# mcosovic/JuliaGrid.jl

Measured on AMD Instinct MI355X. Metric: NR iterations/sec (batched N-1 AC power flow, 10k-bus grid), higher is better.
Workload: dtype f64

## Files before the change

### include/jgrid.h

```cpp
#ifndef JGRID_H
#define JGRID_H

#include <stdint.h>

#ifdef __cplusplus
extern "C" {
#endif

typedef struct jg_nr jg_nr;
typedef struct jg_nr_base jg_nr_base;
typedef struct jg_gn jg_gn;

const char* jg_last_error(void);
int jg_device_count(void);
void jg_plan_cache_clear(void);


int jg_nr_create(jg_nr** h, int64_t n, const int64_t* colptr, const int64_t* rowval,
                 const double* y_reim, const double* yt_reim, const int8_t* type, int64_t slack,
                 int64_t batch, int64_t max_patch, int device);
void jg_nr_destroy(jg_nr* h);

int jg_nr_dims(jg_nr* h, int64_t* dims);

int jg_nr_set_injection(jg_nr* h, const double* p_inj, const double* q_inj, int64_t batch_stride);
int jg_nr_set_voltage(jg_nr* h, const double* vm, const double* va, int64_t batch_stride);
int jg_nr_get_voltage(jg_nr* h, double* vm, double* va);
int jg_nr_snapshot_voltage(jg_nr* h);
int jg_nr_restore_voltage(jg_nr* h);
int jg_nr_get_voltage_device(jg_nr* h, double* vm_dev, double* va_dev);
int jg_nr_pack_results_device(jg_nr* h, double* dst_dev);

int jg_nr_patch_ybus(jg_nr* h, int64_t scenario, int64_t k, const int64_t* ptr, const double* dy_reim);

int jg_nr_patch_ybus_batch(jg_nr* h, int64_t scenario0, int64_t count, int64_t k, const int64_t* ptr, const double* dy_reim);

int jg_nr_set_ybus(jg_nr* h, const double* y_reim, const double* yt_reim);

int jg_nr_mismatch(jg_nr* h, double* max_p, double* max_q);
int jg_nr_solve(jg_nr* h);
int jg_nr_set_refine(jg_nr* h, int mode);
int jg_nr_set_shared(jg_nr* h, int mode);
int jg_nr_run(jg_nr* h, int64_t max_iter, double tol, int32_t* iters, int32_t* status);
int jg_nr_run_defer(jg_nr* h, int64_t max_iter, double tol, int64_t defer_at, int32_t* n_left);
int jg_nr_move_lanes(jg_nr* dst, int64_t dst_lane0, jg_nr* src, int32_t* home, int32_t* count);
int jg_nr_finish(jg_nr* h, int32_t* iters, int32_t* status);
int jg_nr_resume(jg_nr* h, int64_t lanes, int64_t max_iter, double tol, int32_t* iters, int32_t* status);
int jg_nr_pack_rows_device(jg_nr* h, double* dst_dev, int64_t lane0, int64_t count, const int32_t* rows);

int jg_nr_base_create(jg_nr_base** out, jg_nr* single, int64_t top_cap);
void jg_nr_base_destroy(jg_nr_base* b);
int jg_nr_base_info(jg_nr_base* b, int64_t* info);
int jg_nr_base_get(jg_nr_base* b, int which, double* out, int64_t cap);
int jg_nr_attach_base(jg_nr* h, jg_nr_base* b);
int jg_nr_start_from_base(jg_nr* h);
int jg_nr_set_first_iteration(jg_nr* h, int mode);
int jg_nr_first_iteration_counts(jg_nr* h, int64_t* compensated, int64_t* refactorised);

int jg_nr_get_mismatch(jg_nr* h, double* mism);
int jg_nr_get_increment(jg_nr* h, double* incr);
int jg_nr_get_jacobian(jg_nr* h, double* nzval);
int jg_nr_get_maps(jg_nr* h, int64_t* pq, int64_t* pvpq, int64_t* pcount, int64_t* jcolptr, int64_t* jrowval);
int jg_nr_get_iteration(jg_nr* h, int32_t* iters);

int jg_nr_set_bus_type(jg_nr* h, int64_t scenario0, int64_t count, const int8_t* type);
int jg_nr_get_bus_type(jg_nr* h, int8_t* type, int64_t* slack);

int jg_nr_set_generators(jg_nr* h, int64_t ng, const int64_t* bus, const int8_t* status, const double* pg, const double* qmin, const double* qmax,
                         const double* vg, const double* bus_vm, const double* bus_va, const double* pd, const double* qd, double base_mva);
int jg_nr_reactive_limit(jg_nr* h, int flags, int8_t* violate, int32_t* count);
int jg_nr_adjust_angle(jg_nr* h, int64_t bus, double angle);

int jg_nr_fast_setup(jg_nr* h, const double* bp, const double* bq);
int jg_nr_fast_patch_batch(jg_nr* h, int64_t scenario0, int64_t count, int64_t k, const int64_t* ptr, const double* dbp, const double* dbq);
int jg_nr_fast_mismatch(jg_nr* h, double* max_p, double* max_q);
int jg_nr_fast_solve(jg_nr* h);
int jg_nr_fast_run(jg_nr* h, int64_t max_iter, double tol, int32_t* iters, int32_t* status);
int jg_nr_fast_get_increment(jg_nr* h, double* incr);

int jg_nr_set_branches(jg_nr* h, int64_t nb, const int64_t* from, const int64_t* to, const int8_t* status, const double* param);
int jg_nr_set_outage_labels(jg_nr* h, const int64_t* label);
int jg_nr_branch_quantities(jg_nr* h, double* from_pq, double* to_pq, double* series_pq, double* charging_pq,
                            double* from_i, double* to_i, double* series_i);
int jg_nr_bus_injection(jg_nr* h, double* inj_pq);

int jg_nr_set_screen(jg_nr* h, const double* rating);
int jg_nr_screen(jg_nr* h, double* rec);
int jg_nr_screen_device(jg_nr* h, double* rec_dev);
int jg_nr_screen_rows_device(jg_nr* h, double* rec_dev, int64_t lane0, int64_t count, const int32_t* rows);

int jg_nr_time_kernel(jg_nr* h, int kernel, int reps, double* mean_ms);


int jg_gn_create(jg_gn** h, int64_t n, const int64_t* colptr, const int64_t* rowval, const double* y_reim,
                 const double* yt_reim, int64_t nb, const int64_t* from, const int64_t* to, const double* branch_param,
// ... 180 lines not shown
```

### juliagrid.jl_amd/_lib.py

```python
import ctypes as C
import os

import numpy as np

HERE = os.path.dirname(os.path.abspath(__file__))
LIB_PATH = os.environ.get("JG_LIB") or os.path.join(HERE, "libjgrid_hip.so")

I64P = np.ctypeslib.ndpointer(dtype=np.int64, flags="C_CONTIGUOUS")
I32P = np.ctypeslib.ndpointer(dtype=np.int32, flags="C_CONTIGUOUS")
I8P = np.ctypeslib.ndpointer(dtype=np.int8, flags="C_CONTIGUOUS")
F64P = np.ctypeslib.ndpointer(dtype=np.float64, flags="C_CONTIGUOUS")
U8P = np.ctypeslib.ndpointer(dtype=np.uint8, flags="C_CONTIGUOUS")
VP = C.c_void_p

_lib = None


class JGridError(RuntimeError):

    def __init__(self, code, msg):
        super().__init__(f"libjgrid_hip error {code}: {msg}")
        self.code = code


def lib():
    global _lib
    if _lib is not None:
        return _lib
    if not os.path.exists(LIB_PATH):
        raise ImportError(
            f"{LIB_PATH} is missing: build it with `python -c 'import __graft_entry__ as g; g.build()'` "
            "(hipcc --offload-arch=gfx950). There is no CPU fallback.")
    if not os.environ.get("JG_LIB") and not os.environ.get("JG_ALLOW_STALE"):
        from . import build as _build
        if _build.needs_build():
            raise ImportError(f"{LIB_PATH} was not built from the current csrc/ + include/jgrid.h (content hash differs or is missing): rebuild with "
                              "`python -c 'import __graft_entry__ as g; g.build()'`, or set JG_ALLOW_STALE=1 to load it anyway")
    L = C.CDLL(LIB_PATH)
    L.jg_last_error.restype = C.c_char_p
    L.jg_device_count.restype = C.c_int
    sig = {
        "jg_nr_create": [C.POINTER(VP), C.c_int64, I64P, I64P, F64P, F64P, I8P, C.c_int64, C.c_int64, C.c_int64, C.c_int],
        "jg_nr_dims": [VP, I64P],
        "jg_nr_set_injection": [VP, F64P, F64P, C.c_int64],
        "jg_nr_set_voltage": [VP, F64P, F64P, C.c_int64],
        "jg_nr_get_voltage": [VP, F64P, F64P],
        "jg_nr_snapshot_voltage": [VP],
        "jg_nr_restore_voltage": [VP],
        "jg_nr_get_voltage_device": [VP, VP, VP],
        "jg_nr_pack_results_device": [VP, VP],
        "jg_nr_patch_ybus": [VP, C.c_int64, C.c_int64, I64P, F64P],
        "jg_nr_patch_ybus_batch": [VP, C.c_int64, C.c_int64, C.c_int64, I64P, F64P],
        "jg_nr_set_ybus": [VP, F64P, F64P],
        "jg_nr_mismatch": [VP, F64P, F64P],
        "jg_nr_solve": [VP],
        "jg_nr_set_refine": [VP, C.c_int],
        "jg_nr_set_shared": [VP, C.c_int],
        "jg_nr_run": [VP, C.c_int64, C.c_double, I32P, I32P],
        "jg_nr_run_defer": [VP, C.c_int64, C.c_double, C.c_int64, C.POINTER(C.c_int32)],
        "jg_nr_move_lanes": [VP, C.c_int64, VP, I32P, C.POINTER(C.c_int32)],
        "jg_nr_finish": [VP, I32P, I32P],
        "jg_nr_resume": [VP, C.c_int64, C.c_int64, C.c_double, I32P, I32P],
        "jg_nr_pack_rows_device": [VP, VP, C.c_int64, C.c_int64, I32P],
        "jg_nr_get_mismatch": [VP, F64P],
        "jg_nr_get_increment": [VP, F64P],
        "jg_nr_get_jacobian": [VP, F64P],
        "jg_nr_get_maps": [VP, I64P, I64P, I64P, I64P, I64P],
        "jg_nr_get_iteration": [VP, I32P],
        "jg_nr_set_bus_type": [VP, C.c_int64, C.c_int64, VP],
        "jg_nr_get_bus_type": [VP, I8P, I64P],
        "jg_nr_set_generators": [VP, C.c_int64, I64P, I8P, F64P, F64P, F64P, F64P, F64P, F64P, F64P, F64P, C.c_double],
        "jg_nr_reactive_limit": [VP, C.c_int, VP, VP],
        "jg_nr_adjust_angle": [VP, C.c_int64, C.c_double],
        "jg_nr_time_kernel": [VP, C.c_int, C.c_int, C.POINTER(C.c_double)],
        "jg_nr_fast_setup": [VP, F64P, F64P],
        "jg_nr_fast_mismatch": [VP, F64P, F64P],
        "jg_nr_fast_solve": [VP],
        "jg_nr_fast_run": [VP, C.c_int64, C.c_double, I32P, I32P],
        "jg_nr_fast_get_increment": [VP, F64P],
        "jg_nr_set_branches": [VP, C.c_int64, I64P, I64P, I8P, F64P],
        "jg_nr_set_outage_labels": [VP, I64P],
        "jg_nr_branch_quantities": [VP, VP, VP, VP, VP, VP, VP, VP],
        "jg_nr_bus_injection": [VP, F64P],
        "jg_nr_set_screen": [VP, VP],
        "jg_nr_screen": [VP, F64P],
        "jg_nr_screen_device": [VP, VP],
        "jg_nr_screen_rows_device": [VP, VP, C.c_int64, C.c_int64, I32P],
        "jg_gn_create": [C.POINTER(VP), C.c_int64, I64P, I64P, F64P, F64P, C.c_int64, I64P, I64P, F64P, C.c_int64, C.c_int64,
                         I8P, I8P, I64P, C.c_int64, I64P, C.c_int64, C.c_int],
        "jg_gn_dims": [VP, I64P],
        "jg_gn_set_method": [VP, C.c_int],
        "jg_gn_set_measurement": [VP, F64P, F64P, F64P, C.c_int64, C.c_int64],
        "jg_gn_set_voltage": [VP, F64P, F64P, C.c_int64],
        "jg_gn_get_voltage": [VP, F64P, F64P],
        "jg_gn_snapshot_voltage": [VP],
        "jg_gn_restore_voltage": [VP],
        "jg_gn_increment": [VP, F64P],
        "jg_gn_solve": [VP],
        "jg_gn_residual_test": [VP, F64P, I32P],
        "jg_gn_get_normalized_residual": [VP, F64P],
        "jg_gn_evaluate": [VP],
        "jg_gn_set_status": [VP, I8P, I8P],
        "jg_gn_run": [VP, C.c_int64, C.c_double, I32P, I32P],
        "jg_gn_get_maps": [VP, I8P, I64P, I64P],
        "jg_gn_get_jacobian": [VP, F64P],
        "jg_gn_get_residual": [VP, F64P],
        "jg_gn_get_increment": [VP, F64P],
        "jg_gn_get_iteration": [VP, I32P],
        "jg_nr_fast_patch_batch": [VP, C.c_int64, C.c_int64, C.c_int64, I64P, F64P, F64P],
        "jg_gn_set_readings": [VP, C.c_int64, I64P, I8P, F64P, F64P, I8P, F64P, F64P, I8P],
# ... 250 lines not shown
```

### juliagrid.jl_amd/contingency.py

```python
from __future__ import annotations

import queue
import threading
from types import SimpleNamespace as NS

import numpy as np

from . import _lib
from .dcpowerflow import dcContingencyAnalysis
from .pipeline import OrderedRun, gatherBlocks
from .powerflow import (AcPowerFlow, BaseCase, fastNewtonRaphsonBX, fastNewtonRaphsonXB, newtonRaphson, powerFlow_, powerFlowLimits_, setBusType_, setInjection_,
                        setOutages_, startFromBase_, setFirstIteration_, _push_voltage, _upload_branches)
from .system import PowerSystem


def bridges(system: PowerSystem) -> np.ndarray:
    n, nb = system.bus.number, system.branch.number
    f = system.branch.layout.from_ - 1
    t = system.branch.layout.to - 1
    on = np.flatnonzero(system.branch.layout.status == 1)
    adj = [[] for _ in range(n)]
    for k in on:
        adj[f[k]].append((int(t[k]), int(k)))
        adj[t[k]].append((int(f[k]), int(k)))
# ... 187 lines not shown
        while not ev.wait(0.05):
            if run.failed:
                break
            if all(run.solved(i) for i in range(run.nj)):
                self.flush_filling()

    def _serve(self):
        try:
            while True:
                p = self.flush_q.get()
                if p is None:
                    return
                it, st = p.handle.resume(p.fill, self.iteration, self.tolerance)
                for j, home, off in p.routes:
                    result = self.run.wait_solved(j)
                    if result is None:
                        break
                    result[0][home] = it[off:off + home.size]
                    result[1][home] = st[off:off + home.size]
                    if self.record is not None:
                        if self.summary:
                            p.handle.screen_rows_device(self.record(j), off, home)
                        else:
                            p.handle.pack_rows_device(self.record(j), off, home)
                    self.pending[j].set()
                p.clear()
        except BaseException as e:
            self.run.fail(e)


class ContingencyPipeline:

    def __init__(self, system: PowerSystem, batch: int, inflight: int = 3, device: int = 0, start=None, pool: int = 0, defer_at: int = 64,
                 shared_first: bool = True, top_cap: int = 0, reactive_limit: int = 0):
        if reactive_limit and pool:
            raise ValueError("ContingencyPipeline: reactive_limit > 0 with a straggler pool (pool > 0) is not supported")
        if reactive_limit and int(batch) < 2:
            raise ValueError("ContingencyPipeline: reactive_limit needs batches of two or more scenarios")
        self.reactive_limit = max(0, int(reactive_limit))
        self.system, self.batch = system, int(batch)
        self.base = None
        self._shared_first, self._top_cap, self._device = bool(shared_first), int(top_cap), int(device)
        self.handles = [newtonRaphson(system, batch=self.batch, device=device, max_patch=4) for _ in range(max(1, int(inflight)))]
        self.defer_at = max(0, min(64, int(defer_at)))
        self.pools = []
        if pool and self.batch > 64 and self.defer_at > 0:
            lanes = max(2 * self.defer_at, -(-int(pool) // 64) * 64)
            lanes = max(lanes, 256) if -(-self.batch // 64) * 64 >= 256 else min(max(lanes, 128), 192)
            self.pools = [_Pool(newtonRaphson(system, batch=lanes, device=device, max_patch=4)) for _ in range(2)]
        self._stragglers = _StragglerPools(self.pools, self.defer_at) if self.pools else None
        if len(self.handles) + len(self.pools) > 1:
            for an in self.handles + [p.handle for p in self.pools]:
                _lib.check(_lib.lib().jg_nr_set_shared(an._h, 1))
        if start is not None:
            self.setStart(*start)
        else:
            for an in self.handles:
                an.snapshot_voltage()

    def setStart(self, magnitude, angle):
        for an in self.handles:
            _push_voltage(an, magnitude, angle)
            an.snapshot_voltage()
        for p in self.pools:
            _push_voltage(p.handle, magnitude, angle)
        if self.base is not None:
            self.base.close()
            self.base = None
        if self._shared_first and np.ndim(magnitude) == 1:
            single = newtonRaphson(self.system, batch=1, device=self._device)
            _push_voltage(single, magnitude, angle)
            self.base = BaseCase(single, top_cap=self._top_cap)
            single.close()
            for an in self.handles:
                self.base.attach(an)

    def setFirstIteration(self, shared: bool = True):
        for an in self.handles:
            setFirstIteration_(an, shared)

    def close(self):
        for an in self.handles:
            an.close()
        for p in self.pools:
            p.handle.close()
        if self.base is not None:
            self.base.close()
            self.base = None
        self.handles, self.pools, self._stragglers = [], [], None

    def setRating(self, rating):
        r = None if rating is None else np.ascontiguousarray(np.asarray(rating, dtype=np.float64))
        if r is not None and r.shape != (self.system.branch.number,):
            raise ValueError("rating: one value per branch")
        for an in self.handles + [p.handle for p in self.pools]:
            if not an._branches_on_device:
                _upload_branches(an)
            _lib.check(_lib.lib().jg_nr_set_screen(an._h, None if r is None else r.ctypes.data))
            an._screen_rating = r

    def run(self, jobs, iteration: int = 20, tolerance: float = 1e-8, on_done=None, fetch: bool = False, record=None, records: int = 0,
            summary: bool = False):
        jobs = list(jobs)
        pools = self._stragglers
        if pools is not None and on_done is not None and record is None:
            raise ValueError("a pipeline with a straggler pool delivers results through `record`")
# ... 85 lines not shown
```

### juliagrid.jl_amd/csrc/jg_comp.hip

```cpp
#include "jg_comp.hpp"
#include "jg_pf.hpp"

#include <algorithm>
#include <cstdio>
#include <cstdlib>

namespace jg {

namespace {

typedef int RecS __attribute__((ext_vector_type(16)));
typedef const RecS __attribute__((address_space(4)))* RecPtr;
typedef int SegS __attribute__((ext_vector_type(8)));
typedef const SegS __attribute__((address_space(4)))* SegPtr;
typedef const double __attribute__((address_space(4)))* CDbl;
typedef const int __attribute__((address_space(4)))* CInt;
__device__ __forceinline__ RecS load_rec(const Rec* base, size_t index) { return ((RecPtr)base)[index]; }

__device__ __forceinline__ void dsolve(double d00, double d01, double d10, double d11, double r1, double r2, double& y1, double& y2) {
    const bool sw = d10 > 2.0;
    const double l = sw ? d10 - 4.0 : d10;
    const double a = sw ? r2 : r1, b = sw ? r1 : r2;
    y2 = (b - l * a) * d11;
    y1 = (a - d01 * y2) * d00;
}

struct CSweepArgs {
    const Rec* rec; const Segment* seg;
    const double* Mc;
    const double* rhs;
    double* W;
    double* out;
    GroupSel sel; StateUpdate upd;
    int ld, seg_begin, lanes;
    int s0_base, s0_nchunks, s0_wpi, s0_rpw;
};

__device__ __forceinline__ void csweep_record(const CSweepArgs& a, const RecS& r, size_t ld, unsigned off, double& a0, double& a1) {
    static_assert(COMP_T == 6, "operand list of the wait");
    const int nt = r[3];
    d2v w[COMP_T];
#pragma unroll
    for (int t = 0; t < COMP_T; ++t) asm volatile("" : "=v"(w[t]));
#pragma unroll
    for (int t = 0; t < COMP_T; ++t)
        if (t < nt) gload16(w[t], (const char*)a.W + (size_t)r[5 + 2 * t] * ld * 16, off);
    asm volatile("s_waitcnt vmcnt(0)" ::: "memory");
    asm volatile("" : "+v"(w[0]), "+v"(w[1]), "+v"(w[2]), "+v"(w[3]), "+v"(w[4]), "+v"(w[5]));
#pragma unroll
    for (int t = 0; t < COMP_T; ++t)
        if (t < nt) {
            CDbl m = (CDbl)a.Mc + (size_t)r[4 + 2 * t] * 4;
            a0 = fma(-m[1], w[t].y, fma(-m[0], w[t].x, a0));
            a1 = fma(-m[3], w[t].y, fma(-m[2], w[t].x, a1));
        }
}

template <bool BWD>
__global__ __launch_bounds__(512, 4) void k_csweep(CSweepArgs a) {
    extern __shared__ __attribute__((aligned(16))) double red[];
    int base = a.s0_base, nchunks = a.s0_nchunks, wpi = a.s0_wpi, rpw = a.s0_rpw;
    if (blockIdx.y != 0) {
        const SegS sg = ((SegPtr)a.seg)[a.seg_begin + blockIdx.y];
        base = sg[0]; nchunks = sg[1]; wpi = sg[2]; rpw = sg[3];
    }
    int grp, bx;
    if (!map_block(a.sel, a.ld, nchunks * 2, grp, bx)) return;
    const int lane = threadIdx.x;
    const int wave = uniform(threadIdx.y);
    const size_t ld = (size_t)a.ld;
    const size_t b = (size_t)min(grp * 64 + lane, a.lanes - 1);
    const unsigned off = (unsigned)b * 16u;
    const size_t ri = (size_t)base + ((size_t)bx * 8 + wave) * rpw;
    const RecS first = load_rec(a.rec, ri);
    const int sub = wave & (wpi - 1);
    const int k = first[0], src = first[1], dg = first[2];
    double a0 = 0.0, a1 = 0.0;
    int fl = 0; bool act = true; double va = 0.0, vm = 0.0;
    if (k >= 0) {
        if (sub == 0) {
            if (BWD) {
                if (a.upd.va) {
                    act = a.upd.active ? (a.upd.active[b] != 0) : true;
                    fl = uniform((int)a.upd.flags[src]);
                    va = a.upd.va[(size_t)src * ld + b]; vm = a.upd.vm[(size_t)src * ld + b];
                }
                const double2 y = load_vec(a.W, (size_t)k, b, ld);
                CDbl d = (CDbl)a.Mc + (size_t)dg * 4;
                dsolve(d[0], d[1], d[2], d[3], y.x, y.y, a0, a1);
            } else {
                const double2 f = load_vec(a.rhs, (size_t)src, b, ld);
                a0 = f.x; a1 = f.y;
            }
        }
        RecS cur = first;
        for (int j = 1; j < rpw; ++j) {
            const RecS nxt = load_rec(a.rec, ri + j);
            csweep_record(a, cur, ld, off, a0, a1);
            cur = nxt;
        }
        csweep_record(a, cur, ld, off, a0, a1);
        if (wpi > 1 && sub != 0) ((double2*)red)[(size_t)wave * 64 + lane] = double2{a0, a1};
    }
    if (wpi > 1) __syncthreads();
    if (k >= 0 && sub == 0) {
        for (int w = 1; w < wpi; ++w) { const double2 p = ((const double2*)red)[(size_t)(wave + w) * 64 + lane]; a0 += p.x; a1 += p.y; }
        store_vec(a.W, (size_t)k, b, ld, a0, a1);
        if (BWD) {
            if (!a.upd.va || act) store_vec(a.out, (size_t)src, b, ld, a0, a1);
            if (a.upd.va) {
                if (act && (fl & 1)) a.upd.va[(size_t)src * ld + b] = va + a.upd.sign * a0;
                if (act && (fl & 2)) a.upd.vm[(size_t)src * ld + b] = vm + a.upd.sign * a1;
            }
        }
    }
}

constexpr int CTOP_WAVES = 4, CTOP_KPAD = 4 * CTOP_WAVES;
struct CTopArgs {
    const double* Sinv; int n_ks;
    const int* piv; const int* bus;
    double* W; double* out; GroupSel sel; StateUpdate upd;
    int ld, lanes, n, n_top, n_rb;
};
typedef double d4v __attribute__((ext_vector_type(4)));
__global__ __launch_bounds__(64 * CTOP_WAVES) void k_ctop(CTopArgs a) {
    __shared__ double part[CTOP_WAVES][4][4][64];
    int grp, rb;
    if (!map_block(a.sel, a.ld, a.n_rb, grp, rb)) return;
    const int lane = threadIdx.x;
    const int wave = uniform(threadIdx.y);
    const size_t ld = (size_t)a.ld;
    const int kq = lane >> 4, col = lane & 15;
    size_t boff[4];
#pragma unroll
    for (int j = 0; j < 4; ++j) boff[j] = (size_t)min(grp * 64 + 16 * j + col, a.lanes - 1) * 2 + (kq & 1);
    const double* y = a.W + ((size_t)a.n + (kq >> 1)) * ld * 2;
    const double* sa = a.Sinv + ((size_t)rb * a.n_ks) * 64 + lane;
    d4v acc[4];
#pragma unroll
    for (int j = 0; j < 4; ++j) acc[j] = d4v{0.0, 0.0, 0.0, 0.0};
    const int per = a.n_ks / CTOP_WAVES;
    const int k0 = wave * per, k1 = k0 + per;
    constexpr int U = 4;
    for (int ks = k0; ks < k1; ks += U) {
        double av[U], bv[U][4];
#pragma unroll
        for (int u = 0; u < U; ++u) {
            const int kk = min(ks + u, k1 - 1);
            av[u] = sa[(size_t)kk * 64];
            const double* yr = y + (size_t)(2 * kk) * ld * 2;
#pragma unroll
            for (int j = 0; j < 4; ++j) bv[u][j] = yr[boff[j]];
        }
#pragma unroll
        for (int u = 0; u < U; ++u)
            if (ks + u < k1) {
#pragma unroll
                for (int j = 0; j < 4; ++j) acc[j] = __builtin_amdgcn_mfma_f64_16x16x4f64(av[u], bv[u][j], acc[j], 0, 0, 0);
            }
    }
#pragma unroll
    for (int j = 0; j < 4; ++j)
#pragma unroll
        for (int r = 0; r < 4; ++r) part[wave][j][r][lane] = acc[j][r];
    __syncthreads();
    const int j = wave;
    const int lb = grp * 64 + 16 * j + col;
    if (lb >= a.lanes) return;
    const size_t b = (size_t)lb;
    const bool act = a.upd.va ? (a.upd.active ? (a.upd.active[b] != 0) : true) : true;
    const int c = kq & 1;
#pragma unroll
    for (int r = 0; r < 4; ++r) {
        const int t = 8 * rb + (kq >> 1) + 2 * r;
        double x = 0.0;
#pragma unroll
        for (int w = 0; w < CTOP_WAVES; ++w) x += part[w][j][r][lane];
        if (t >= a.n_top) continue;
        const int k = a.piv[t], bus = a.bus[t];
        a.W[((size_t)k * ld + b) * 2 + c] = x;
        if (!a.upd.va || act) a.out[((size_t)bus * ld + b) * 2 + c] = x;
        if (a.upd.va && act) {
            const int fl = (int)a.upd.flags[bus];
            double* st = c == 0 ? a.upd.va : a.upd.vm;
            if (fl & (1 << c)) st[(size_t)bus * ld + b] += a.upd.sign * x;
        }
    }
}

__global__ void k_comp_pack(const double* X, int ldx, const int* e_row, const int* e_col, const int* diag, double* Mc, int n_entries) {
    const int e = blockIdx.x * blockDim.x + threadIdx.x;
    if (e >= n_entries) return;
    auto blk = [&](int id, double (&v)[4]) {
        const double* p = X + (size_t)id * 4 * ldx;
        v[0] = p[0]; v[1] = p[1]; v[2] = p[(size_t)2 * ldx]; v[3] = p[(size_t)2 * ldx + 1];
    };
    const int r = e_row[e], c = e_col[e];
    double x[4], d[4], o[4];
    blk(e, x);
    if (r == c) { o[0] = x[0]; o[1] = x[1]; o[2] = x[2]; o[3] = x[3]; }
    else if (r > c) {
        blk(diag[c], d);
        const bool sw = d[2] > 2.0;
        const double l = sw ? d[2] - 4.0 : d[2];
        const double z1 = x[0] * d[0], w1 = x[2] * d[0];
        const double z2 = (x[1] - z1 * d[1]) * d[3], w2 = (x[3] - w1 * d[1]) * d[3];
        const double y1 = z1 - z2 * l, v1 = w1 - w2 * l;
        if (sw) { o[0] = z2; o[1] = y1; o[2] = w2; o[3] = v1; } else { o[0] = y1; o[1] = z2; o[2] = v1; o[3] = w2; }
    } else {
        blk(diag[r], d);
        dsolve(d[0], d[1], d[2], d[3], x[0], x[2], o[0], o[2]);
        dsolve(d[0], d[1], d[2], d[3], x[1], x[3], o[1], o[3]);
    }
    double* m = Mc + (size_t)e * 4;
    m[0] = o[0]; m[1] = o[1]; m[2] = o[2]; m[3] = o[3];
}

__global__ void k_unit_rhs(double* rhs, const int* row, const int* comp, int ld, int count) {
    const int b = blockIdx.x * blockDim.x + threadIdx.x;
    if (b >= count || row[b] < 0) return;
    rhs[((size_t)row[b] * ld + b) * 2 + comp[b]] = 1.0;
}
__global__ void k_unit_clear(double* rhs, const int* row, const int* comp, int ld, int count) {
    const int b = blockIdx.x * blockDim.x + threadIdx.x;
    if (b >= count || row[b] < 0) return;
    rhs[((size_t)row[b] * ld + b) * 2 + comp[b]] = 0.0;
}
__global__ void k_take_sinv(const double* W, const int* piv, double* Sinv, int n_ks, int n_top, int ld, int col0, int count) {
    const int b = blockIdx.x * blockDim.x + threadIdx.x, i = blockIdx.y;
    if (b >= count || i >= n_top) return;
    const double2 x = *(const double2*)(W + ((size_t)piv[i] * ld + b) * 2);
    const int kc = col0 + b, ks = kc >> 2, kq = kc & 3;
    for (int c = 0; c < 2; ++c) {
        const int r = 2 * i + c, rb = r >> 4, rr = r & 15;
        Sinv[((size_t)rb * n_ks + ks) * 64 + kq * 16 + rr] = c ? x.y : x.x;
    }
}
__global__ void k_take_z(const double* out, const int* bus, const int* comp, const int* rowptr, const int* colm, const int* tpos, double* Zc, int ld, int count) {
    const int b = blockIdx.x * blockDim.x + threadIdx.x;
    if (b >= count || bus[b] < 0) return;
    const int a = bus[b], c = comp[b];
    for (int p = rowptr[a]; p < rowptr[a + 1]; ++p) {
        const int j = colm[p] & 0xffffff;
        const double2 x = *(const double2*)(out + ((size_t)j * ld + b) * 2);
        double* z = Zc + (size_t)tpos[p] * 4;
        z[c] = x.x; z[2 + c] = x.y;
    }
}

struct Fix4 { double m[4][4]; };
__global__ __launch_bounds__(64) void k_comp_fix(CompFixArgs a) {
    const int b = blockIdx.x * 64 + threadIdx.x;
    if (b >= a.lanes) return;
    if (a.active && !a.active[b]) return;
    int pos[8]; double dg[8], db[8];
    int ne = 0;
    for (int m = 0; m < a.mp; ++m) {
        const int p = a.ppos[(size_t)m * a.ld + b];
        if (p < 0) continue;
        pos[ne] = p; dg[ne] = a.pdg[(size_t)m * a.ld + b]; db[ne] = a.pdb[(size_t)m * a.ld + b]; ++ne;
    }
    if (ne == 0) return;
    int ba = a.posrow[pos[0]], bb = -1;
    for (int e = 0; e < ne; ++e) {
        const int i = a.posrow[pos[e]], j = a.colm[pos[e]] & 0xffffff;
        if (i != ba && bb < 0) bb = i;
        if (j != ba && bb < 0) bb = j;
    }
    const bool two = bb >= 0;
    if (two && bb < ba) { const int t = ba; ba = bb; bb = t; }
    if (!two) bb = ba;
    const int bus[2] = {ba, bb};
    double v[2], th[2]; int ty[2];
    for (int s = 0; s < 2; ++s) { v[s] = a.v0[bus[s]]; th[s] = a.th0[bus[s]]; ty[s] = a.rowtype[bus[s]] & 3; }
    double M[4][4] = {{0.0}}, ds1[2] = {0.0, 0.0}, ds2[2] = {0.0, 0.0}, dgii[2] = {0.0, 0.0}, dbii[2] = {0.0, 0.0};
    for (int e = 0; e < ne; ++e) {
        const int i = a.posrow[pos[e]], cm = a.colm[pos[e]], j = cm & 0xffffff, mk = cm >> 24;
        const int si = i == ba ? 0 : 1, sj = j == ba ? 0 : 1;
        double sn, cs;
        sincos(th[si] - th[sj], &sn, &cs);
        const pf::Terms t = pf::entry_terms(dg[e], db[e], sn, cs);
        ds1[si] += v[sj] * t.ac; ds2[si] += v[sj] * t.ad;
        if (i == j) { dgii[si] = dg[e]; dbii[si] = db[e]; continue; }
        const Blk o = pf::offdiag(mk, v[si], v[sj], t.ac, t.ad);
// ... 21 lines not shown
        double t = (two || s == 0) ? a.y0[2 * bus[s] + (r & 1)] : 0.0;
        for (int c = 0; c < 4; ++c) t += S[r][c] * df[c];
        w[r] = t;
        for (int c = 0; c < 4; ++c) {
            double q = r == c ? 1.0 : 0.0;
            for (int k = 0; k < 4; ++k) q += S[r][k] * M[k][c];
            A[r][c] = q;
        }
    }
    double ref[4];
    for (int r = 0; r < 4; ++r) { ref[r] = 0.0; for (int c = 0; c < 4; ++c) ref[r] = fmax(ref[r], fabs(A[r][c])); }
    bool bad = false;
    for (int k = 0; k < 4; ++k) {
        int piv = k;
        for (int r = k + 1; r < 4; ++r) if (fabs(A[r][k]) > fabs(A[piv][k])) piv = r;
        if (piv != k) {
            for (int c = 0; c < 4; ++c) { const double t = A[k][c]; A[k][c] = A[piv][c]; A[piv][c] = t; }
            { const double t = w[k]; w[k] = w[piv]; w[piv] = t; }
            { const double t = ref[k]; ref[k] = ref[piv]; ref[piv] = t; }
        }
        if (!(fabs(A[k][k]) > PIVOT_EPS * ref[k])) bad = true;
        const double ip = 1.0 / A[k][k];
        for (int r = k + 1; r < 4; ++r) {
            const double l = A[r][k] * ip;
            for (int c = k + 1; c < 4; ++c) A[r][c] -= l * A[k][c];
            w[r] -= l * w[k];
        }
    }
    double u[4];
    for (int k = 3; k >= 0; --k) {
        double t = w[k];
        for (int c = k + 1; c < 4; ++c) t -= A[k][c] * u[c];
        u[k] = t / A[k][k];
    }
    if (bad || !(fabs(u[0]) < 1.0e300) || !(fabs(u[1]) < 1.0e300) || !(fabs(u[2]) < 1.0e300) || !(fabs(u[3]) < 1.0e300)) { atomicOr(a.lu_status + b, 4); return; }
    for (int s = 0; s < (two ? 2 : 1); ++s) {
        double c0 = 0.0, c1 = 0.0;
        for (int k = 0; k < 4; ++k) { c0 += M[2 * s][k] * u[k]; c1 += M[2 * s + 1][k] * u[k]; }
        double* f = a.F + ((size_t)bus[s] * a.ld + b) * 2;
        f[0] -= c0; f[1] -= c1;
    }
}

}

void launch_comp_fix(const CompFixArgs& a, hipStream_t st) {
    hipLaunchKernelGGL(k_comp_fix, dim3((unsigned)((a.lanes + 63) / 64)), dim3(64), 0, st, a);
}

int CompSweep::upload_tables(const BlockSymbolic& S, int top_cap, hipStream_t st, std::string& err) {
    build_comp_tables(S, top_cap, T);
    std::vector<int> bus(T.top.size());
    for (size_t i = 0; i < T.top.size(); ++i) bus[i] = S.perm[T.top[i]];
    if (upload(&fwd_rec, T.fwd_rec, err, st) || upload(&fwd_seg, T.fwd_seg, err, st) || upload(&bwd_rec, T.bwd_rec, err, st) || upload(&bwd_seg, T.bwd_seg, err, st) ||
        upload(&top_piv, T.top, err, st) || upload(&top_bus, bus, err, st)) return 2;
    auto launches = [](const std::vector<Segment>& segs, std::vector<DevLaunch>& out) {
        out.clear();
        size_t s = 0;
        while (s < segs.size()) {
            DevLaunch d{};
            d.seg_begin = (int)s;
            while (true) {
                d.nseg++; d.grid = std::max(d.grid, segs[s].nchunks); d.wpi_max = std::max(d.wpi_max, segs[s].wpi);
                if (segs[s++].last) break;
            }
            d.seg_end = (int)s;
            out.push_back(d);
        }
    };
    launches(T.fwd_seg, fwd);
    launches(T.bwd_seg, bwd);
    return 0;
}

void CompSweep::free_tables() {
    hipFree(fwd_rec); hipFree(fwd_seg); hipFree(bwd_rec); hipFree(bwd_seg); hipFree(top_piv); hipFree(top_bus);
    fwd_rec = bwd_rec = nullptr; fwd_seg = bwd_seg = nullptr; top_piv = top_bus = nullptr;
}

int CompBase::solve(const CompSweep& sw, hipStream_t st, const double* rhs, double* Wc, double* out, int ld, int lanes, const StateUpdate& upd, const GroupSel& sel) const {
    CSweepArgs a{sw.fwd_rec, sw.fwd_seg, Mc, rhs, Wc, out, sel, StateUpdate{}, ld, 0, lanes, 0, 0, 1, 1};
    for (const DevLaunch& L : sw.fwd) {
        a.seg_begin = L.seg_begin;
        { const Segment& g = sw.T.fwd_seg[L.seg_begin]; a.s0_base = g.rec_base; a.s0_nchunks = g.nchunks; a.s0_wpi = g.wpi; a.s0_rpw = g.rpw; }
        hipLaunchKernelGGL((k_csweep<false>), dim3(grid_blocks(ld / 64, (long long)L.grid * 2), L.nseg), dim3(64, 8), 8 * 64 * sizeof(double2), st, a);
    }
    if (sw.T.n_top > 0) {
        const int n_rb = (2 * sw.T.n_top + 15) / 16;
        CTopArgs t{Sinv, lds, sw.top_piv, sw.top_bus, Wc, out, sel, upd, ld, lanes, n, sw.T.n_top, n_rb};
        hipLaunchKernelGGL(k_ctop, dim3(grid_blocks(ld / 64, n_rb)), dim3(64, CTOP_WAVES), 0, st, t);
    }
    a.rec = sw.bwd_rec; a.seg = sw.bwd_seg; a.upd = upd;
    for (const DevLaunch& L : sw.bwd) {
        a.seg_begin = L.seg_begin;
        { const Segment& g = sw.T.bwd_seg[L.seg_begin]; a.s0_base = g.rec_base; a.s0_nchunks = g.nchunks; a.s0_wpi = g.wpi; a.s0_rpw = g.rpw; }
        hipLaunchKernelGGL((k_csweep<true>), dim3(grid_blocks(ld / 64, (long long)L.grid * 2), L.nseg), dim3(64, 8), 8 * 64 * sizeof(double2), st, a);
    }
    if (hipGetLastError() != hipSuccess) return 2;
    return 0;
}

#define CB_HIP(expr)                                                                      \
    do {                                                                                  \
        hipError_t err__ = (expr);                                                        \
        if (err__ != hipSuccess) { error = std::string(#expr) + ": " + hipGetErrorString(err__); return 2; } \
    } while (0)

int CompBase::create(const BlockSymbolic& S, const double* Xsrc, int ldx, int top_cap, hipStream_t st) {
    if (S.symmetric) { error = "the shared-factor solve is built for unsymmetric plans (the Newton-Raphson Jacobian)"; return 1; }
    n = S.n; n_entries = S.n_entries;
    CB_HIP(hipGetDevice(&device));
    if (full.upload_tables(S, -1, st, error)) return 2;
    if (split.upload_tables(S, top_cap, st, error)) return 2;
    {
        int* d_row = nullptr; int* d_col = nullptr; int* d_diag = nullptr;
        if (upload(&d_row, S.e_row, error, st) || upload(&d_col, S.e_col, error, st) || upload(&d_diag, S.diag, error, st)) { hipFree(d_row); hipFree(d_col); hipFree(d_diag); return 2; }
        hipError_t e = hipMalloc((void**)&Mc, (size_t)n_entries * 4 * sizeof(double));
        if (e == hipSuccess) {
            hipLaunchKernelGGL(k_comp_pack, dim3((n_entries + 255) / 256), dim3(256), 0, st, Xsrc, ldx, (const int*)d_row, (const int*)d_col, (const int*)d_diag, Mc, n_entries);
            e = hipStreamSynchronize(st);
        }
        hipFree(d_row); hipFree(d_col); hipFree(d_diag);
        CB_HIP(e);
    }
    const int nt = split.T.n_top;
    if (nt > 0) {
        const int n_rb = (2 * nt + 15) / 16;
        lds = (2 * nt + CTOP_KPAD - 1) / CTOP_KPAD * (CTOP_KPAD / 4);
        const size_t sbytes = (size_t)n_rb * lds * 64 * sizeof(double);
        CB_HIP(hipMalloc((void**)&Sinv, sbytes));
        CB_HIP(sync_fill(Sinv, 0, sbytes, st));
        const int ldb = 512;
        double* rhs = nullptr; double* W = nullptr; double* out = nullptr; int* d_rowi = nullptr; int* d_comp = nullptr;
        const size_t vec = (size_t)n * ldb * 2 * sizeof(double);
        hipError_t e = hipMalloc((void**)&rhs, vec);
        if (e == hipSuccess) e = hipMalloc((void**)&W, vec);
        if (e == hipSuccess) e = hipMalloc((void**)&out, vec);
        if (e == hipSuccess) e = hipMalloc((void**)&d_rowi, ldb * sizeof(int));
        if (e == hipSuccess) e = hipMalloc((void**)&d_comp, ldb * sizeof(int));
        if (e == hipSuccess) e = sync_fill(rhs, 0, vec, st);
        std::vector<int> hr(ldb), hc(ldb);
        for (int c0 = 0; e == hipSuccess && c0 < 2 * nt; c0 += ldb) {
// ... 60 lines not shown
```

### juliagrid.jl_amd/csrc/jg_comp.hpp

```cpp
#pragma once
#include "jg_engine.hpp"

namespace jg {

struct CompSweep {
    CompTables T;
    Rec* fwd_rec = nullptr; Segment* fwd_seg = nullptr; Rec* bwd_rec = nullptr; Segment* bwd_seg = nullptr;
    int* top_piv = nullptr; int* top_bus = nullptr;
    std::vector<DevLaunch> fwd, bwd;
    int upload_tables(const BlockSymbolic& S, int top_cap, hipStream_t st, std::string& err);
    void free_tables();
};

struct CompBase {
    int n = 0, nnz = 0, n_entries = 0, device = 0;
    CompSweep full, split;
    double* Mc = nullptr;
    double* Sinv = nullptr; int lds = 0;
    double* Zc = nullptr;
    double* v0 = nullptr; double* th0 = nullptr; double* f0 = nullptr; double* y0 = nullptr;
    double* p0 = nullptr; double* q0 = nullptr;
    int* rowptr = nullptr; int* colm = nullptr; int* posrow = nullptr; int* tpos = nullptr; int* rowtype = nullptr;
    std::string error;

    int create(const BlockSymbolic& S, const double* Xsrc, int ldx, int top_cap, hipStream_t st);
    void destroy();
    int solve(const CompSweep& sw, hipStream_t st, const double* rhs, double* Wc, double* out, int ld, int lanes, const StateUpdate& upd, const GroupSel& sel) const;
    size_t scratch_rows(const CompSweep& sw) const { return (size_t)n + (size_t)((sw.T.n_top + 7) & ~7); }
};

struct CompFixArgs {
    const int* ppos; const double* pdg; const double* pdb; int mp;
    const int* rowptr; const int* colm; const int* posrow; const int* rowtype;
    const double* v0; const double* th0; const double* y0; const double* Zc;
    double* F; int* lu_status; const int* active;
    int ld, lanes;
};
void launch_comp_fix(const CompFixArgs& a, hipStream_t st);
int comp_form_z(CompBase& B, hipStream_t st);

}
```

### juliagrid.jl_amd/csrc/jg_engine.hip

```cpp
#include "jg_engine.hpp"

#include <algorithm>
#include <chrono>
#include <cstdio>
#include <cstdlib>
#include <condition_variable>
#include <mutex>

namespace jg {

namespace {

struct FactArgs {
    const Rec* rec; const Segment* seg;
    const double* A; const double* rhs; double* X; double* W; int* status; GroupSel sel;
    int ld, seg_begin;
    int lanes;
    int s0_base, s0_nchunks, s0_wpi, s0_rpw;
};

struct BwdArgs {
    const Rec* rec; const Segment* seg; const int* chain;
    const double* X; double* W; double* out; GroupSel sel;
    StateUpdate upd;
    int ld, seg_begin;
    int lanes;
    int s0_base, s0_nchunks, s0_wpi, s0_rpw;
};


__device__ __forceinline__ void dsolve(const Blk& d, double r1, double r2, double& y1, double& y2) {
    const bool sw = d.v10 > 2.0;
    const double l = sw ? d.v10 - 4.0 : d.v10;
    const double a = sw ? r2 : r1, b = sw ? r1 : r2;
    y2 = (b - l * a) * d.v11;
    y1 = (a - d.v01 * y2) * d.v00;
}

__device__ __forceinline__ void term3(Blk& c, const Blk& l, const Blk& d, const Blk& u) {
    double z00, z10, z01, z11;
    dsolve(d, u.v00, u.v10, z00, z10);
    dsolve(d, u.v01, u.v11, z01, z11);
    c.v00 -= l.v00 * z00 + l.v01 * z10;
    c.v01 -= l.v00 * z01 + l.v01 * z11;
    c.v10 -= l.v10 * z00 + l.v11 * z10;
    c.v11 -= l.v10 * z01 + l.v11 * z11;
}

typedef int RecS __attribute__((ext_vector_type(16)));
typedef const RecS __attribute__((address_space(4)))* RecPtr;
__device__ __forceinline__ RecS load_rec(const Rec* base, size_t index) { return ((RecPtr)base)[index]; }
__device__ __forceinline__ int rec_word(const RecS& r, int k) { return r[k]; }


__device__ __forceinline__ void fact_record(const FactArgs& a, const RecS& r, int kind, size_t b, size_t ld, Blk& c) {
    static_assert(FACT_T == 4, "operand list of the wait");
    const int nt = rec_word(r, 3);
    BlkV l[FACT_T], d[FACT_T], u[FACT_T];
#pragma unroll
    for (int t = 0; t < FACT_T; ++t) asm volatile("" : "=v"(l[t].r0), "=v"(l[t].r1), "=v"(d[t].r0), "=v"(d[t].r1), "=v"(u[t].r0), "=v"(u[t].r1));
    const char* const usrc = kind == 3 ? (const char*)a.W : (const char*)a.X;
    const size_t urow = kind == 3 ? ld * 16 : ld * 32, uhalf = kind == 3 ? 0 : ld * 16;
    const unsigned off = (unsigned)b * 16u;
#pragma unroll
    for (int t = 0; t < FACT_T; ++t) {
        if (t < nt) {
            const char* pl = (const char*)a.X + (size_t)(rec_word(r, 4 + 3 * t) & 0x3fffffff) * ld * 32;
            const char* pd = (const char*)a.X + (size_t)rec_word(r, 5 + 3 * t) * ld * 32;
            const char* pu = usrc + (size_t)rec_word(r, 6 + 3 * t) * urow;
            gload16(l[t].r0, pl, off); gload16(l[t].r1, pl + ld * 16, off);
            gload16(d[t].r0, pd, off); gload16(d[t].r1, pd + ld * 16, off);
            gload16(u[t].r0, pu, off); gload16(u[t].r1, pu + uhalf, off);
        }
    }
    {
        asm volatile("s_waitcnt vmcnt(0)" ::: "memory");
        asm volatile("" : "+v"(l[0].r0), "+v"(l[0].r1), "+v"(d[0].r0), "+v"(d[0].r1), "+v"(u[0].r0), "+v"(u[0].r1),
                          "+v"(l[1].r0), "+v"(l[1].r1), "+v"(d[1].r0), "+v"(d[1].r1), "+v"(u[1].r0), "+v"(u[1].r1));
        asm volatile("" : "+v"(l[2].r0), "+v"(l[2].r1), "+v"(d[2].r0), "+v"(d[2].r1), "+v"(u[2].r0), "+v"(u[2].r1),
                          "+v"(l[3].r0), "+v"(l[3].r1), "+v"(d[3].r0), "+v"(d[3].r1), "+v"(u[3].r0), "+v"(u[3].r1));
// ... 49 lines not shown
            const RecS nxt = load_rec(a.rec, rec_index + j);
            fact_record(a, cur, kind, b, ld, c);
            cur = nxt;
        }
        fact_record(a, cur, kind, b, ld, c);
        if (wpi > 1 && sub != 0) {
            double2* q = (double2*)red + (size_t)wave * 128 + lane;
            q[0] = double2{c.v00, c.v01}; q[64] = double2{c.v10, c.v11};
        }
    }
    if (wpi > 1) __syncthreads();
    if (kind >= 0 && sub == 0) {
        for (int w = 1; w < wpi; ++w) {
            const double2* q = (const double2*)red + (size_t)(wave + w) * 128 + lane;
            const double2 h0 = q[0], h1 = q[64];
            c.v00 += h0.x; c.v01 += h0.y; c.v10 += h1.x; c.v11 += h1.y;
        }
        fact_finish(a, kind, id, b, ld, c, ref);
    }
    if (wpi > 1) __syncthreads();
}

__device__ __forceinline__ void bwd_record(const BwdArgs& a, const RecS& r, size_t b, size_t ld, double& y0, double& y1) {
    const int nt = rec_word(r, 3);
    Blk m[BWD_T]; double w0[BWD_T], w1[BWD_T];
#pragma unroll
    for (int t = 0; t < BWD_T; ++t) {
        if (t < nt) {
            m[t] = load_blk(a.X, (size_t)rec_word(r, 4 + 2 * t), b, ld);
            const double2 w = load_vec(a.W, (size_t)rec_word(r, 5 + 2 * t), b, ld);
            w0[t] = w.x; w1[t] = w.y;
        }
    }
#pragma unroll
    for (int t = 0; t < BWD_T; ++t) {
        if (t < nt) {
            y0 -= m[t].v00 * w0[t] + m[t].v01 * w1[t];
            y1 -= m[t].v10 * w0[t] + m[t].v11 * w1[t];
        }
    }
}

struct UpdPre { int fl; bool act; double va, vm; };
__device__ __forceinline__ UpdPre upd_prefetch(const BwdArgs& a, int bus, size_t b, size_t ld) {
    UpdPre p{0, false, 0.0, 0.0};
    if (a.upd.va) {
        p.act = a.upd.active ? (a.upd.active[b] != 0) : true;
        p.fl = uniform((int)a.upd.flags[bus]);
        p.va = a.upd.va[(size_t)bus * ld + b];
        p.vm = a.upd.vm[(size_t)bus * ld + b];
    }
    return p;
}
__device__ __forceinline__ double2 bwd_finish(const BwdArgs& a, const Blk& d, double y0, double y1, int k, int bus, size_t b, size_t ld, const UpdPre& p) {
    double x0, x1;
    dsolve(d, y0, y1, x0, x1);
    store_vec(a.W, (size_t)k, b, ld, x0, x1);
    if (!a.upd.va || p.act) store_vec(a.out, (size_t)bus, b, ld, x0, x1);
    if (a.upd.va) {
        if (p.act && (p.fl & 1)) a.upd.va[(size_t)bus * ld + b] = p.va + a.upd.sign * x0;
        if (p.act && (p.fl & 2)) a.upd.vm[(size_t)bus * ld + b] = p.vm + a.upd.sign * x1;
    }
    return double2{x0, x1};
}

constexpr int CHAIN_PF = 3;
typedef const int __attribute__((address_space(4)))* CIntPtr;
constexpr int CHAIN_LDS_D2 = (CHAIN_MAX_ROWS + CHAIN_MAX_EXT + 16 + 2) * 64;

__device__ __forceinline__ void bwd_chain_task(const BwdArgs& a, double* lds, const RecS& rec, int wave, int lane, size_t b, size_t ld) {
    const int nb = rec[0], nE = rec[1], wpr = rec[3];
    CIntPtr rows = (CIntPtr)a.chain + rec[2];
    CIntPtr ecol = rows + 3 * nb;
    CIntPtr uext = ecol + nE;
    CIntPtr uin = uext + nb * nE;
    double2* acc = (double2*)lds;
    double2* xe = acc + CHAIN_MAX_ROWS * 64;
    double2* part = xe + CHAIN_MAX_EXT * 64;
    double2* xc = part + 16 * 64;
    for (int q = wave; q < nE; q += 16) xe[q * 64 + lane] = load_vec(a.W, (size_t)ecol[q], b, ld);
    UpdPre up0{0, false, 0.0, 0.0}, up1{0, false, 0.0, 0.0};
    if (wave < nb) up0 = upd_prefetch(a, rows[3 * wave + 1], b, ld);
    if (wave + 16 < nb) up1 = upd_prefetch(a, rows[3 * (wave + 16) + 1], b, ld);
    __syncthreads();
    const int rpr = 16 / wpr, sub = wave & (wpr - 1);
    const int len = (nE + wpr - 1) / wpr;
    for (int p0 = 0; p0 < nb; p0 += rpr) {
        const int p = p0 + wave / wpr;
        double y0 = 0.0, y1 = 0.0;
        if (p < nb) {
            if (sub == 0) { const double2 y = load_vec(a.W, (size_t)rows[3 * p], b, ld); y0 = y.x; y1 = y.y; }
            const int q1 = min(sub * len + len, nE);
            for (int q = sub * len; q < q1; q += 4) {
                Blk m[4];
#pragma unroll
                for (int t = 0; t < 4; ++t) if (q + t < q1) m[t] = load_blk(a.X, (size_t)uext[p * nE + q + t], b, ld);
#pragma unroll
                for (int t = 0; t < 4; ++t)
                    if (q + t < q1) {
                        const double2 x = xe[(q + t) * 64 + lane];
                        y0 -= m[t].v00 * x.x + m[t].v01 * x.y;
                        y1 -= m[t].v10 * x.x + m[t].v11 * x.y;
                    }
            }
        }
        if (wpr > 1) {
            part[wave * 64 + lane] = double2{y0, y1};
            __syncthreads();
            if (p < nb && sub == 0) for (int w = 1; w < wpr; ++w) { const double2 t = part[(wave + w) * 64 + lane]; y0 += t.x; y1 += t.y; }
        }
        if (p < nb && sub == 0) acc[p * 64 + lane] = double2{y0, y1};
        if (wpr > 1) __syncthreads();
    }
    __syncthreads();
    Blk mb[CHAIN_PF][2], db[CHAIN_PF];
    auto request = [&](int c, Blk (&m)[2], Blk& d) {
        if (c < 0) return;
        if (wave == (c & 15)) d = load_blk(a.X, (size_t)rows[3 * c + 2], b, ld);
#pragma unroll
        for (int i = 0; i < 2; ++i) { const int p = wave + 16 * i; if (p < c) m[i] = load_blk(a.X, (size_t)uin[p * nb + c], b, ld); }
    };
#pragma unroll
    for (int s = 0; s < CHAIN_PF; ++s) request(nb - 1 - s, mb[s], db[s]);
    for (int c0 = nb - 1; c0 >= 0; c0 -= CHAIN_PF) {
#pragma unroll
        for (int s = 0; s < CHAIN_PF; ++s) {
            const int c = c0 - s;
            if (c >= 0) {
                double2* slot = xc + (c & 1) * 64;
                if (wave == (c & 15)) {
                    const double2 y = acc[c * 64 + lane];
                    slot[lane] = bwd_finish(a, db[s], y.x, y.y, rows[3 * c], rows[3 * c + 1], b, ld, c < 16 ? up0 : up1);
                }
                __syncthreads();
                const double2 x = slot[lane];
#pragma unroll
                for (int i = 0; i < 2; ++i) {
                    const int p = wave + 16 * i;
                    if (p < c) {
                        double2 t = acc[p * 64 + lane];
                        t.x -= mb[s][i].v00 * x.x + mb[s][i].v01 * x.y;
                        t.y -= mb[s][i].v10 * x.x + mb[s][i].v11 * x.y;
                        acc[p * 64 + lane] = t;
                    }
                }
                request(c - CHAIN_PF, mb[s], db[s]);
            }
        }
    }
    __syncthreads();
}

constexpr int CHAIN_SMALL_LDS_D2 = (8 + 2) * 64;
__device__ __forceinline__ void bwd_chain_small(const BwdArgs& a, double* lds, const RecS& rec, int wave, int lane, size_t b, size_t ld) {
    const int nb = rec[0], nE = rec[1], wpr = rec[3];
    CIntPtr rows = (CIntPtr)a.chain + rec[2];
    CIntPtr ecol = rows + 3 * nb;
    CIntPtr uext = ecol + nE;
    CIntPtr uin = uext + nb * nE;
    double2* part = (double2*)lds;
    double2* xc = part + 8 * 64;
    const int p = wave / wpr, sub = wave & (wpr - 1);
    const bool live = wave < 8 && p < nb, owner = live && sub == 0;
    UpdPre up{0, false, 0.0, 0.0};
    double y0 = 0.0, y1 = 0.0;
    Blk d{0.0, 0.0, 0.0, 0.0};
    int k = 0, bus = 0;
    Blk mb[CHAIN_PF];
    auto request = [&](int c, Blk& m) { if (owner && c > p) m = load_blk(a.X, (size_t)uin[p * nb + c], b, ld); };
    if (owner) {
        k = rows[3 * p]; bus = rows[3 * p + 1];
        up = upd_prefetch(a, bus, b, ld);
        const double2 y = load_vec(a.W, (size_t)k, b, ld); y0 = y.x; y1 = y.y;
        d = load_blk(a.X, (size_t)rows[3 * p + 2], b, ld);
    }
#pragma unroll
    for (int s = 0; s < CHAIN_PF; ++s) request(nb - 1 - s, mb[s]);
    if (live) {
        const int len = (nE + wpr - 1) / wpr;
        const int q1 = min(sub * len + len, nE);
        for (int q = sub * len; q < q1; q += 4) {
            Blk m[4]; double2 x[4];
#pragma unroll
            for (int t = 0; t < 4; ++t)
                if (q + t < q1) { m[t] = load_blk(a.X, (size_t)uext[p * nE + q + t], b, ld); x[t] = load_vec(a.W, (size_t)ecol[q + t], b, ld); }
#pragma unroll
            for (int t = 0; t < 4; ++t)
                if (q + t < q1) {
                    y0 -= m[t].v00 * x[t].x + m[t].v01 * x[t].y;
                    y1 -= m[t].v10 * x[t].x + m[t].v11 * x[t].y;
                }
        }
    }
    if (wpr > 1) {
        if (live && sub != 0) part[wave * 64 + lane] = double2{y0, y1};
        __syncthreads();
        if (owner) for (int w = 1; w < wpr; ++w) { const double2 t = part[(wave + w) * 64 + lane]; y0 += t.x; y1 += t.y; }
    }
    for (int c0 = nb - 1; c0 >= 0; c0 -= CHAIN_PF) {
#pragma unroll
        for (int s = 0; s < CHAIN_PF; ++s) {
            const int c = c0 - s;
            if (c >= 0) {
                double2* slot = xc + (c & 1) * 64;
                if (owner && p == c) slot[lane] = bwd_finish(a, d, y0, y1, k, bus, b, ld, up);
                if (c > 0) {
                    __syncthreads();
                    if (owner && p < c) {
                        const double2 x = slot[lane];
                        y0 -= mb[s].v00 * x.x + mb[s].v01 * x.y;
                        y1 -= mb[s].v10 * x.x + mb[s].v11 * x.y;
                    }
                    request(c - CHAIN_PF, mb[s]);
                }
            }
        }
    }
}

__device__ __forceinline__ void bwd_chunk(const BwdArgs& a, double* red, const RecS& first, size_t rec_index, int rpw, int wpi,
                                          int wave, int lane, size_t b, size_t ld) {
    const int sub = wave & (wpi - 1);
    const int k = rec_word(first, 0), bus = rec_word(first, 1), dg = rec_word(first, 2);
    double y0 = 0.0, y1 = 0.0;
    Blk d{0.0, 0.0, 0.0, 0.0};
    UpdPre up{0, false, 0.0, 0.0};
    if (k >= 0) {
        if (sub == 0) {
            up = upd_prefetch(a, bus, b, ld);
            const double2 y = load_vec(a.W, (size_t)k, b, ld);
            y0 = y.x; y1 = y.y;
            d = load_blk(a.X, (size_t)dg, b, ld);
        }
        RecS cur = first;
        for (int j = 1; j < rpw; ++j) {
            const RecS nxt = load_rec(a.rec, rec_index + j);
            bwd_record(a, cur, b, ld, y0, y1);
            cur = nxt;
        }
        bwd_record(a, cur, b, ld, y0, y1);
        if (wpi > 1 && sub != 0) ((double2*)red)[(size_t)wave * 64 + lane] = double2{y0, y1};
    }
    if (wpi > 1) __syncthreads();
    if (k >= 0 && sub == 0) {
        for (int w = 1; w < wpi; ++w) { const double2 p = ((const double2*)red)[(size_t)(wave + w) * 64 + lane]; y0 += p.x; y1 += p.y; }
        bwd_finish(a, d, y0, y1, k, bus, b, ld, up);
    }
    if (wpi > 1) __syncthreads();
}

typedef int SegS __attribute__((ext_vector_type(8)));
typedef const SegS __attribute__((address_space(4)))* SegPtr;

template <bool BWD, int BW = 16, class Args>
__device__ __forceinline__ void level_body(const Args& a, double* red) {
    int base = a.s0_base, nchunks = a.s0_nchunks, wpi = a.s0_wpi, rpw = a.s0_rpw;
    if (blockIdx.y != 0) {
        const SegS sg = ((SegPtr)a.seg)[a.seg_begin + blockIdx.y];
        base = sg[0]; nchunks = sg[1]; wpi = sg[2]; rpw = sg[3];
    }
    int grp, bx;
    if (!map_block(a.sel, a.ld, BWD ? (wpi <= 0 ? nchunks : nchunks * (16 / BW)) : nchunks * (16 / FACT_WAVES), grp, bx)) return;
    const int lane = threadIdx.x;
    const int wave = uniform(threadIdx.y);
    const size_t ld = (size_t)a.ld;
    const size_t b = (size_t)min(grp * 64 + lane, a.lanes - 1);
    if constexpr (BWD) {
        if (wpi <= 0) {
            if (wpi < 0) bwd_chain_small(a, red, load_rec(a.rec, (size_t)base + bx), wave, lane, b, ld);
            else if constexpr (BW == 16) bwd_chain_task(a, red, load_rec(a.rec, (size_t)base + bx), wave, lane, b, ld);
            return;
        }
    }
    const size_t ri = (size_t)base + ((size_t)bx * (BWD ? BW : FACT_WAVES) + wave) * rpw;
    const RecS r = load_rec(a.rec, ri);
    if constexpr (BWD) bwd_chunk(a, red, r, ri, rpw, wpi, wave, lane, b, ld);
    else fact_chunk(a, red, r, ri, rpw, wpi, wave, lane, b, ld);
}

__global__ __launch_bounds__(64 * FACT_WAVES, 4) void k_fact_level(FactArgs a) {
    extern __shared__ __attribute__((aligned(16))) double red[];
    level_body<false>(a, red);
}

__global__ __launch_bounds__(1024) void k_bwd_level(BwdArgs a) {
    extern __shared__ __attribute__((aligned(16))) double red[];
    level_body<true>(a, red);
}

__global__ __launch_bounds__(512, 4) void k_bwd_level8(BwdArgs a) {
    extern __shared__ __attribute__((aligned(16))) double red[];
    level_body<true, 8>(a, red);
}

struct Bwd1Args {
    const int* t_row; const int* t_ptr; const int* t_term; const int* t_level;
    const int* b_wg; const int* b_row; const int* b_term;
    const double* X; const double* jc; double* W; double* out; GroupSel sel; StateUpdate upd;
    int ld, n_top_levels, n_wg, n_top;
// ... 1384 lines not shown

void clear_plan_cache() {
    std::lock_guard<std::mutex> lock(g_plan_mutex);
    g_plans.clear();
}

std::shared_ptr<SharedPlan> acquire_plan(int n, const int* rowptr, const int* col, long long policy, hipStream_t st, std::string& error, int& rc) {
    rc = 0;
    int device = 0;
    if (hipGetDevice(&device) != hipSuccess) { error = "no HIP device"; rc = 2; return nullptr; }
    if (n <= 0 || !rowptr || !col || rowptr[0] != 0) { error = "block pattern must be structurally symmetric with a full diagonal"; rc = 1; return nullptr; }
    static const bool nocache = knob("PLAN_CACHE", 1) == 0;
    const unsigned long long h = pattern_hash(n, rowptr, col, policy, device);
    struct Pending { unsigned long long hash; long long policy; int device, n; };
    static std::vector<Pending>* pending = new std::vector<Pending>();
    static std::condition_variable* pending_cv = new std::condition_variable();
    auto is_pending = [&] { for (const Pending& q : *pending) if (q.hash == h && q.policy == policy && q.device == device && q.n == n) return true; return false; };
    std::unique_lock<std::mutex> lock(g_plan_mutex);
    for (;;) {
        if (!nocache)
            for (size_t i = 0; i < g_plans.size(); ++i) {
                const std::shared_ptr<SharedPlan>& p = g_plans[i];
                if (p->key_hash == h && p->device == device && p->policy == policy && p->S.n == n && (int)p->key_col.size() == rowptr[n] &&
                    std::equal(rowptr, rowptr + n + 1, p->key_rowptr.begin()) && std::equal(col, col + rowptr[n], p->key_col.begin())) {
                    std::shared_ptr<SharedPlan> hit = p;
                    g_plans.erase(g_plans.begin() + i);
                    g_plans.push_back(hit);
                    return hit;
                }
            }
        if (nocache || !is_pending()) break;
        pending_cv->wait(lock);
    }
    if (!nocache) pending->push_back(Pending{h, policy, device, n});
    lock.unlock();
    struct Done {
        std::unique_lock<std::mutex>& lock; std::vector<Pending>* pending; std::condition_variable* cv; unsigned long long h; long long policy; int device, n; bool armed;
        ~Done() {
            if (!armed) return;
            if (!lock.owns_lock()) lock.lock();
            for (size_t i = 0; i < pending->size(); ++i)
                if ((*pending)[i].hash == h && (*pending)[i].policy == policy && (*pending)[i].device == device && (*pending)[i].n == n) { pending->erase(pending->begin() + i); break; }
            cv->notify_all();
        }
    } done{lock, pending, pending_cv, h, policy, device, n, !nocache};
    std::shared_ptr<SharedPlan> p = std::make_shared<SharedPlan>();
    if (analyze(n, rowptr, col, policy, p->S)) { error = "block pattern must be structurally symmetric with a full diagonal"; rc = 1; return nullptr; }
    p->device = device; p->policy = policy; p->key_hash = h;
    p->key_rowptr.assign(rowptr, rowptr + n + 1); p->key_col.assign(col, col + rowptr[n]);
    const BlockSymbolic& S = p->S;
    const double tu0 = std::chrono::duration<double, std::milli>(std::chrono::steady_clock::now().time_since_epoch()).count();
    std::vector<int> prow(n, 0);
    for (int k = 0; k < n; ++k) if (S.prefactor && S.pre_pivot[k]) prow[S.perm[k]] = k + 1;
    if (upload(&p->pre_rec, S.pre_rec, error, st) || upload(&p->pre_seg, S.pre_seg, error, st) || upload(&p->pre_row, prow, error, st) ||
        upload(&p->fact_rec, S.fact_rec, error, st) || upload(&p->bwd_rec, S.bwd_rec, error, st) || upload(&p->fact_seg, S.fact_seg, error, st) ||
        upload(&p->bwd_seg, S.bwd_seg, error, st) || upload(&p->bwd_chain, S.bwd_chain, error, st) ||
        (S.jordan && (upload(&p->bwdj_rec, S.bwdj_rec, error, st) || upload(&p->bwdj_seg, S.bwdj_seg, error, st))) ||
        upload(&p->fwd_rec, S.fwd_rec, error, st) || upload(&p->fwd_seg, S.fwd_seg, error, st) ||
        (S.single_fact_ok && (upload(&p->f1_rec, S.f_rec, error, st) || upload(&p->f1_wg, S.f1_wg, error, st))) ||
        (!S.top_launch.empty() && (upload(&p->top_task, S.top_task, error, st) || upload(&p->top_data, S.top_data, error, st) || upload(&p->top_wgmap, S.top_wgmap, error, st)))) {
        rc = 2;
        return nullptr;
    }
    if (knob_set("PLAN_TIMING")) fprintf(stderr, "[jg engine]   table upload %6.1f ms\n", std::chrono::duration<double, std::milli>(std::chrono::steady_clock::now().time_since_epoch()).count() - tu0);
    if (!nocache) {
        lock.lock();
        g_plans.push_back(p);
        size_t idle = 0;
        for (const auto& q : g_plans) if (q.use_count() == 1) ++idle;
        for (size_t i = 0; i < g_plans.size() && idle > PLAN_CACHE_KEEP;)
            if (g_plans[i].use_count() == 1) { g_plans.erase(g_plans.begin() + i); --idle; } else ++i;
    }
    return p;
}

int Engine::create(int n, const int* rowptr, const int* col, int ld_, long long policy, hipStream_t st) {
    if (ld_ <= 0 || ld_ % 64) { error = "batch leading dimension must be a positive multiple of 64"; return 1; }
    const bool defaults = !((policy >> 16) & 0x7fff);
    if (defaults && ld_ >= 256) policy |= 8;
    {
        static const int tasks_env = knob("ROW_TASKS", 1);
        if (defaults && !((policy >> 32) & 0xff) && (tasks_env == 2 || (tasks_env == 1 && ld_ >= 256))) policy |= 1LL << 50;
    }
    constexpr bool top_r02 = false;
    const bool tiny = !top_r02 && ld_ == 64 && lanes > 0 && lanes <= 32 && !(policy & 2);
    const bool lane64 = !top_r02 && ld_ == 64 && !tiny && n >= 4000 && !(policy & 2);
    if (defaults) policy |= ld_ >= 256 ? (n >= 4000 ? (top_r02 || (policy & 2) ? (47 << 16 | (384 / 8) << 24 | 8 << 4) : (47 << 16 | 127 << 24 | 12 << 4)) : (47 << 16 | (280 / 8) << 24 | 4 << 4))
                                              : ((n >= 4000 ? 26 : 24) << 16 | (tiny || lane64 ? 127 : 384 / 8) << 24 | (lane64 ? 15 << 4 : 0));
    if (defaults && tiny && !((policy >> 54) & 0x3f)) policy |= 12LL << 54;
    if (defaults && tiny && lanes == 1 && knob("SINGLE", 1) != 0) policy |= 1LL << 60;
    const bool timing = knob_set("PLAN_TIMING");
    auto tnow = [] { return std::chrono::duration<double, std::milli>(std::chrono::steady_clock::now().time_since_epoch()).count(); };
    const double te0 = tnow();
    {
        int rc = 0;
        plan = acquire_plan(n, rowptr, col, policy, st, error, rc);
        if (!plan) return rc;
    }
    if (timing) fprintf(stderr, "[jg engine] plan (analysis or cache hit, table upload) %6.1f ms\n", tnow() - te0);
    ld = ld_;
    level_launches(plan->S.fact_seg, fact);
    level_launches(plan->S.pre_seg, pre);
    level_launches(plan->S.bwd_seg, bwd);
    level_launches(plan->S.bwdj_seg, bwdj);
    level_launches(plan->S.fwd_seg, fwd);
    jordan = plan->S.jordan && knob("JORDAN", 1) != 0;
    if (ld == 64 && lanes == 1 && jordan && knob("SINGLE", 1) != 0) {
        std::lock_guard<std::mutex> lock(plan->single_mutex);
        if (!plan->single_tried) {
            plan->single_tried = true;
// ... 180 lines not shown
        }
        level_launches(plan->S.sel_seg, selv);
        sel_rec = plan->sel_rec; sel_seg = plan->sel_seg;
        JG_HIP(hipMalloc((void**)&Zs, factor_bytes()));
        JG_HIP(sync_fill(Zs, 0, factor_bytes(), st));
    }
    SelArgs a{sel_rec, sel_seg, X, Zs, sel, ld, 0, lanes > 0 ? lanes : ld, 0, 0, 1, 1};
    for (const DevLaunch& L : selv) {
        a.seg_begin = L.seg_begin;
        { const Segment& g = plan->S.sel_seg[L.seg_begin]; a.s0_base = g.rec_base; a.s0_nchunks = g.nchunks; a.s0_wpi = g.wpi; a.s0_rpw = g.rpw; }
        hipLaunchKernelGGL(k_sel_level, dim3(grid_blocks(ld / 64, (long long)L.grid * (16 / FACT_WAVES)), L.nseg), dim3(64, FACT_WAVES), FACT_WAVES * 128 * sizeof(double2), st, a);
    }
    JG_HIP(hipGetLastError());
    return 0;
}

int Engine::forward(hipStream_t st, const double* rhs, const GroupSel& sel) {
    FactArgs a{fwd_rec, fwd_seg, X, rhs, X, W, status, sel, ld, 0, lanes > 0 ? lanes : ld, 0, 0, 1, 1};
    for (const DevLaunch& L : fwd) {
        a.seg_begin = L.seg_begin;
        { const Segment& g = plan->S.fwd_seg[L.seg_begin]; a.s0_base = g.rec_base; a.s0_nchunks = g.nchunks; a.s0_wpi = g.wpi; a.s0_rpw = g.rpw; }
        hipLaunchKernelGGL(k_fact_level, dim3(grid_blocks(ld / 64, (long long)L.grid * (16 / FACT_WAVES)), L.nseg), dim3(64, FACT_WAVES), FACT_WAVES * 256 * sizeof(double), st, a);
    }
    JG_HIP(hipGetLastError());
    return 0;
}

namespace {
__global__ void k_fill_shared(const double* blocks, const int* src_entry, double* X, int nnz, int ld) {
    const int p = blockIdx.x * blockDim.y + threadIdx.y;
    if (p >= nnz) return;
    const size_t b = (size_t)blockIdx.y * 64 + threadIdx.x;
    const double* v = blocks + (size_t)p * 4;
    store_blk(X, (size_t)src_entry[p], b, (size_t)ld, v[0], v[1], v[2], v[3]);
}
}

int Engine::set_shared_matrix(hipStream_t st, const double* blocks_host) {
    if (!plan->S.inplace) { error = "set_shared_matrix needs an in-place engine"; return 1; }
    const int nnz = (int)plan->S.src_entry.size();
    double* dblk = nullptr; int* dmap = nullptr;
    std::vector<double> hb(blocks_host, blocks_host + (size_t)nnz * 4);
    if (upload(&dblk, hb, error, st) || upload(&dmap, plan->S.src_entry, error, st)) { hipFree(dblk); hipFree(dmap); return 2; }
    hipLaunchKernelGGL(k_fill_shared, dim3((nnz + 3) / 4, ld / 64), dim3(64, 4), 0, st, dblk, dmap, X, nnz, ld);
    hipError_t e = hipStreamSynchronize(st);
    hipFree(dblk); hipFree(dmap);
    JG_HIP(e);
    return 0;
}

int Engine::backsolve(hipStream_t st, double* out, const StateUpdate& upd, const GroupSel& sel) {
    if (single_bwd && jordan) {
        const SingleTables& T = plan->single;
        Bwd1Args s{plan->s1_t_row, plan->s1_t_ptr, plan->s1_t_term, plan->s1_t_level, plan->s1_b_wg, plan->s1_b_row, plan->s1_b_term, X, jc, W, out, sel, upd, ld, T.n_top_levels, T.n_wg, T.n_top,
                   plan->s1_t_jb, plan->s1_t_cslot, plan->s1_t_toff, T.max_level_terms};
        const int flat_env = knob("SINGLE", 1);
        if (T.flat_ok && flat_env != 2) hipLaunchKernelGGL(k_bwd1_top2, dim3(grid_blocks(ld / 64, 1)), dim3(1024), (size_t)T.n_top * 36 + (size_t)T.max_level_terms * 16, st, s);
        else hipLaunchKernelGGL(k_bwd1_top, dim3(grid_blocks(ld / 64, 1)), dim3(1024), (size_t)T.n_top * 40, st, s);
        if (T.n_wg > 0) hipLaunchKernelGGL(k_bwd1_bottom, dim3(grid_blocks(ld / 64, T.n_wg)), dim3(SINGLE_BOTTOM_ROWS), 0, st, s);
        JG_HIP(hipGetLastError());
        return 0;
    }
    BwdArgs a{jordan ? plan->bwdj_rec : bwd_rec, jordan ? plan->bwdj_seg : bwd_seg, bwd_chain, X, W, out, sel, upd, ld, 0, lanes > 0 ? lanes : ld, 0, 0, 1, 1};
    const std::vector<Segment>& segs = jordan ? plan->S.bwdj_seg : plan->S.bwd_seg;
    for (const DevLaunch& L : (jordan ? bwdj : bwd)) {
        a.seg_begin = L.seg_begin;
        { const Segment& g = segs[L.seg_begin]; a.s0_base = g.rec_base; a.s0_nchunks = g.nchunks; a.s0_wpi = g.wpi; a.s0_rpw = g.rpw; }
        if (!L.chain && L.wpi_max <= 8)
            hipLaunchKernelGGL(k_bwd_level8, dim3(grid_blocks(ld / 64, (long long)L.grid * 2), L.nseg), dim3(64, 8), CHAIN_SMALL_LDS_D2 * sizeof(double2), st, a);
        else
        hipLaunchKernelGGL(k_bwd_level, dim3(grid_blocks(ld / 64, L.grid), L.nseg), dim3(64, 16),
                           L.chain ? (size_t)CHAIN_LDS_D2 * sizeof(double2) : 16 * 128 * sizeof(double), st, a);
    }
    JG_HIP(hipGetLastError());
    return 0;
}

}
```

### juliagrid.jl_amd/csrc/jg_nr.hip

```cpp
#include <hip/hip_runtime.h>

#include <algorithm>
#include <atomic>
#include <chrono>
#include <cmath>
#include <cstdio>
#include <cstdlib>
#include <cstring>
#include <mutex>
#include <string>
#include <system_error>
#include <thread>
#include <type_traits>
#include <vector>

#include "../../include/jgrid.h"
#include "jg_engine.hpp"
#include "jg_pf.hpp"
#include "jg_comp.hpp"
#include "jg_compact.hpp"
#include "jg_lanes.hpp"
#include "jg_qlim.hpp"

namespace {
// ... 442 lines not shown
        }
    }
    red[0][wave][lane] = mp;
    red[1][wave][lane] = mq;
    __syncthreads();
    if (wave != 0) return;
    for (int w = 1; w < 16; ++w) {
        mp = pf::nanmax(red[0][w][lane], mp); mq = pf::nanmax(red[1][w][lane], mq);
    }
    a.normp[b] = mp;
    a.normq[b] = mq;
    if (a.mode == 0) return;
    const double tol = a.params[0];
    const int maxit = (int)a.params[1];
    const jg::Verdict v = jg::verdict(mp < tol && mq < tol, a.lu_status[b], mp != mp || mq != mq, a.iters + b, maxit, b < a.batch);
    a.active[b] = v.go ? 1 : 0;
    a.status[b] = v.status;
    if (v.go) { a.iters[b] += 1; atomicAdd(a.counter, 1); }
}

__global__ __launch_bounds__(256) void k_pack_rows(const double* vm, const double* va, const int* iters, const int* status, const int* rows,
                                                   double* dst, int n, int ld, int lane0, long long stride) {
    const int i = blockIdx.y;
    const int b = lane0 + i;
    double* out = dst + (size_t)rows[i] * stride;
    for (int j = blockIdx.x * 256 + threadIdx.x; j < n; j += gridDim.x * 256) { out[j] = vm[(size_t)j * ld + b]; out[n + j] = va[(size_t)j * ld + b]; }
    if (blockIdx.x == 0 && threadIdx.x == 0) { out[2 * n] = (double)iters[b]; out[2 * n + 1] = (double)status[b]; }
}

}

namespace jg {
void set_last_error(const std::string& msg) { g_error = msg; }
}

struct jg_nr : jg::Lanes {
    int n = 0, nnz = 0, mp = 0, device = 0, nchunk = 0;
    int64_t dimJ = 0, nnzJ = 0, slack = 0;
    std::vector<int64_t> colptr, rowval, pq, pvpq, pcount, jcolptr, jrowval;
    std::vector<int8_t> type;
    std::vector<int> tperm;
    std::vector<int64_t> jmap;
    int* d_rowptr = nullptr; int* d_col = nullptr; double* d_G = nullptr; double* d_B = nullptr; double2* d_GB = nullptr; int* d_rowtype = nullptr; int* d_rowtype_pre = nullptr;
    signed char* d_type = nullptr; signed char* d_flags = nullptr;
    double* d_vm = nullptr; double* d_va = nullptr; double* d_p = nullptr; double* d_q = nullptr;
    int* d_ppos = nullptr; double* d_pdg = nullptr; double* d_pdb = nullptr;
    int* d_dst = nullptr; double* d_F = nullptr; double* d_inc = nullptr; double* d_part = nullptr;
    double* d_normp = nullptr; double* d_normq = nullptr; double* d_params = nullptr;
    double* d_vm0 = nullptr; double* d_va0 = nullptr;
    int* d_active = nullptr; int* d_iters = nullptr; int* d_status = nullptr; int* d_counter = nullptr; int* d_group = nullptr;
    int* d_lid = nullptr; int* d_dest = nullptr; int* d_cflags = nullptr; int* d_itmp = nullptr; int* d_glist = nullptr;
    jg::Compaction cmp{};
    bool refine = false;
    bool fast = false;
    std::vector<double> fast_blk;
    std::vector<int> fp_entry; std::vector<double> fp_dp, fp_dq;
    int* d_fp_entry = nullptr; double* d_fp_dp = nullptr; double* d_fp_dq = nullptr;
    double* d_R = nullptr;
    double* d_inc2[2] = {nullptr, nullptr};
    const int* fast_mask = nullptr;
    jg::Graph gFA, gFB;
    int nb = 0;
    int* d_bfrom = nullptr; int* d_bto = nullptr; signed char* d_bstatus = nullptr; double* d_bparam = nullptr; int* d_outage = nullptr;
    double* d_post = nullptr; size_t post_bytes = 0;
    double* d_rating = nullptr; double* d_screen = nullptr; double* d_screc = nullptr;
    jg::Engine eng;
    jg::Graph gA, gB, gBm, gJ;
    jg::Graph gM; int m_iters = 0;
    int stop_hint = 0, iter_graphs = 0;
    long long last_guess_hit = 0, last_guess_miss = 0;
    bool jac_valid = false;
    bool level0_done = false;
    bool f_stale = false;
    bool paused = false;
    int* d_move = nullptr;
    int* h_move = nullptr;
    double host_launch_us = 0.0, host_wait_us = 0.0; long long host_iters = 0;
    bool res_pinned = false;
    int* h_counter_dev = nullptr;
    std::vector<int> csr_row, csr_col;
    jg_nr_base* base = nullptr;
    double* d_cw = nullptr;
    bool start_is_base = false;
    int first_mode = 1;
    std::vector<unsigned char> patch_state;
    bool inj_checked = false, inj_equal = false;
    int* d_cmp = nullptr;
    jg::Graph gA2, gC;
    long long first_comp = 0, first_full = 0;
    unsigned long long* d_lt = nullptr;
    signed char* d_flags_all = nullptr;
    std::vector<unsigned char> lt_set;
    std::vector<unsigned char> dead;
    bool lt_on = false;
    jg::QlimTables qt;
    int* d_skip = nullptr;
    double* d_shift = nullptr;
};

struct jg_nr_base {
    jg::CompBase cb;
    int n = 0, nnz = 0, device = 0;
    std::vector<int64_t> colptr, rowval;
    std::vector<int8_t> type;
    hipStream_t stream = nullptr;
    std::atomic<int> refs{1};
    double create_ms = 0.0;
};

namespace {

int set_device(jg_nr* h) { NR_HIP(hipSetDevice(h->device)); return 0; }

unsigned char classify_patch(const jg_nr* h, const int* pos, int k) {
    int a = -1, b = -1;
    bool any = false, joined = false;
    for (int m = 0; m < k; ++m) {
        if (pos[m] < 0) continue;
        any = true;
        const int ij[2] = {h->csr_row[pos[m]], h->csr_col[pos[m]]};
        for (int q = 0; q < 2; ++q) {
            if (a < 0 || ij[q] == a) a = ij[q];
            else if (b < 0 || ij[q] == b) b = ij[q];
            else return 2;
        }
        if (ij[0] != ij[1]) joined = true;
    }
    if (!any) return 0;
    return (b < 0 || joined) ? 1 : 2;
}

jg::GroupSel active_groups(jg_nr* h) { return jg::GroupSel{nullptr, h->d_glist, h->d_cflags + jg::CF_LIST}; }

template <class F> void with_mp(int mp, F&& f) {
    switch (mp) {
        case 0: f(std::integral_constant<int, 0>{}); break;
        case 4: f(std::integral_constant<int, 4>{}); break;
        default: f(std::integral_constant<int, 8>{}); break;
    }
}
template <class F> void with_mp_jac(int mp, bool jac, F&& f) {
    with_mp(mp, [&](auto m) { if (jac) f(m, std::true_type{}); else f(m, std::false_type{}); });
}

void launch_assemble(jg_nr* h, const jg::GroupSel& sel = jg::GroupSel{}, bool jac = true, double* pq_out = nullptr, int fd_mode = 0, const int* only_if = nullptr,
                     bool level0 = false) {
    const bool pre = jac && level0 && h->eng.plan->S.prefactor && h->d_rowtype_pre;
    AsmArgs a{h->d_rowptr, h->d_col, h->d_GB, pre ? h->d_rowtype_pre : h->d_rowtype, h->d_dst, h->d_vm, h->d_va, h->d_p, h->d_q,
              h->d_ppos, h->d_pdg, h->d_pdb, h->eng.X, h->d_F, h->d_part, pq_out, sel, fd_mode ? h->d_R : nullptr, fd_mode, h->n, h->ld, h->mp, h->nchunk, h->batch, only_if,
              h->eng.W, h->eng.status, h->lt_on ? h->d_lt : nullptr};
    if (jac && !only_if) h->level0_done = pre;
    const bool lt = h->lt_on;
    dim3 grid(jg::grid_blocks(h->ld / 64, h->nchunk)), block(64, ASM_WAVES);
    auto go = [&](auto kernel, dim3 g, dim3 b) { hipLaunchKernelGGL(kernel, g, b, 0, h->stream, a); };
    const bool single_env = jg::knob("SINGLE", 1) != 0;
    if (h->ld == 64 && h->batch == 1 && !fd_mode && !pq_out && !only_if && single_env) {
        const dim3 g1(jg::grid_blocks(1, (h->n + 63) / 64));
        with_mp_jac(h->mp, jac, [&](auto m, auto j) { go(k_assemble1<decltype(m)::value, decltype(j)::value>, g1, dim3(256)); });
        return;
    }
    if (h->ld == 64 && h->batch <= 32 && !fd_mode && !pq_out) {
        const bool w16 = h->nchunk <= 512;
        const dim3 wide(64, w16 ? 16 : 8);
        with_mp_jac(h->mp, jac, [&](auto m, auto j) {
            constexpr int MP = decltype(m)::value; constexpr bool JAC = decltype(j)::value;
            if (lt) { if (w16) go(k_assemble<MP, JAC, 16, true>, grid, wide); else go(k_assemble<MP, JAC, 8, true>, grid, wide); }
            else { if (w16) go(k_assemble<MP, JAC, 16, false>, grid, wide); else go(k_assemble<MP, JAC, 8, false>, grid, wide); }
        });
        return;
    }
    with_mp_jac(h->mp, jac, [&](auto m, auto j) {
        constexpr int MP = decltype(m)::value; constexpr bool JAC = decltype(j)::value;
        if (lt) go(k_assemble<MP, JAC, ASM_WAVES, true>, grid, block); else go(k_assemble<MP, JAC>, grid, block);
    });
}

__global__ __launch_bounds__(1024) void k_verdict64(CheckArgs a, jg::CompactArgs p) {
    __shared__ double red[2][16][64];
    const int lane = threadIdx.x, wave = threadIdx.y;
    const int b = lane;
    const int grp_on = a.group ? a.group[0] : 1;
    const double tol = a.params[0];
    const int maxit = (int)a.params[1];
    const int lus = a.lu_status[b], its = a.iters[b], act0 = a.active[b], st0 = a.status[b];
// ... 12 lines not shown
            double x[CU], y[CU];
#pragma unroll
            for (int u = 0; u < CU; ++u) {
                const int c = min(c0 + 16 * u, a.nchunk - 1);
                x[u] = a.part[((size_t)c * 2) * a.ld + b]; y[u] = a.part[((size_t)c * 2 + 1) * a.ld + b];
            }
#pragma unroll
            for (int u = 0; u < CU; ++u) { mp = pf::nanmax(x[u], mp); mq = pf::nanmax(y[u], mq); }
        }
        red[0][wave][lane] = mp;
        red[1][wave][lane] = mq;
    }
    __syncthreads();
    if (wave != 0) return;
    const bool skip = grp_on == 0;
    int act = act0, it_out = its, st_out = st0;
    if (!skip) {
        const int src = a.batch == 1 ? 0 : lane;
        for (int w = a.batch == 1 ? 0 : 1; w < 16; ++w) { mp = pf::nanmax(red[0][w][src], mp); mq = pf::nanmax(red[1][w][src], mq); }
        a.normp[b] = mp;
        a.normq[b] = mq;
        const jg::Verdict v = jg::verdict(mp < tol && mq < tol, lus, mp != mp || mq != mq, &its, maxit, b < a.batch);
        act = v.go ? 1 : 0;
        a.active[b] = act;
        st_out = v.status;
        a.status[b] = st_out;
        if (v.go) { it_out = its + 1; a.iters[b] = it_out; atomicAdd(a.counter, 1); }
    }
    const int n_active = __popcll(__ballot(act != 0));
    if (p.host_res && n_active == 0) { p.host_res[lane] = it_out; p.host_res[64 + lane] = st_out; __threadfence_system(); }
    if (lane == 0) {
        p.flags[0] = 0; p.flags[1] = n_active; p.flags[4] = 0;
        p.group[0] = n_active > 0 ? 1 : 0;
        if (n_active > 0) p.glist[0] = 0;
        p.flags[3] = n_active > 0 ? 1 : 0;
        if (p.host_count) *p.host_count = n_active;
    }
}

CheckArgs check_args(jg_nr* h, const int* group, int mode) {
    return CheckArgs{h->d_part, h->nchunk, h->ld, h->batch, h->d_params, h->d_normp, h->d_normq, h->d_active, h->d_iters, h->d_status, h->eng.status, h->d_counter, group, mode};
}
void launch_verdict64(jg_nr* h, bool report) {
    hipLaunchKernelGGL(k_verdict64, dim3(1), dim3(64, 16), 0, h->stream, check_args(h, h->d_group, 1), h->cmp.args(0, report));
}

void launch_check(jg_nr* h, int mode, const int* group = nullptr) {
    hipLaunchKernelGGL(k_check, dim3(h->ld / 64), dim3(64, 16), 0, h->stream, check_args(h, group, mode));
}

void launch_compact(jg_nr* h, int restore, bool report = false) {
    std::vector<jg::LaneRows> rows{{h->d_vm, h->n, 1}, {h->d_va, h->n, 1}, {h->d_p, h->n, 1}, {h->d_q, h->n, 1}};
    if (h->mp > 0) { rows.push_back({h->d_pdg, h->mp, 1}); rows.push_back({h->d_pdb, h->mp, 1}); }
    rows.push_back({h->d_inc, h->n, 2});
    if (h->lt_on) rows.push_back({(double*)h->d_lt, (h->n + 31) / 32, 1});
    h->cmp.launch_compact(h->stream, restore, report, rows);
}

int newton_step(jg_nr* h, const jg::GroupSel& sel, const int* active) {
    if (int rc = h->eng.factor(h->stream, nullptr, h->d_F, sel, h->level0_done)) return rc;
    if (!h->refine) {
        jg::StateUpdate upd{h->d_va, h->d_vm, h->lt_on ? h->d_flags_all : h->d_flags, active, -1.0};
        return h->eng.backsolve(h->stream, h->d_inc, upd, sel);
    }
    jg::StateUpdate none{};
    if (int rc = h->eng.backsolve(h->stream, h->d_inc2[1], none, sel)) return rc;
    RefineArgs a{h->d_rowptr, h->d_col, h->d_GB, h->d_rowtype, h->d_vm, h->d_va, h->d_ppos, h->d_pdg, h->d_pdb,
                 h->d_F, h->d_inc2[1], h->d_R, sel, h->n, h->ld, h->mp, h->nchunk, h->batch};
    dim3 grid(jg::grid_blocks(h->ld / 64, h->nchunk)), block(64, ASM_WAVES);
    with_mp(h->mp, [&](auto m) { hipLaunchKernelGGL((k_refine_residual<decltype(m)::value>), grid, block, 0, h->stream, a); });
    if (int rc = h->eng.forward(h->stream, h->d_R, sel)) return rc;
    if (int rc = h->eng.backsolve(h->stream, h->d_inc2[0], none, sel)) return rc;
    hipLaunchKernelGGL(k_refine_apply, dim3(jg::grid_blocks(h->ld / 64, (h->n + 15) / 16)), dim3(64, 16), 0, h->stream,
                       h->d_inc, h->d_inc2[1], h->d_inc2[0], h->d_va, h->d_vm, h->d_flags, active, sel, h->n, h->ld, h->batch);
    return 0;
}

int build_graphs(jg_nr* h) {
    if (h->gA) return 0;
    auto check_and_compact = [&]() {
        if (h->ld == 64) { launch_verdict64(h, true); return; }
        launch_check(h, 1, h->d_group);
        launch_compact(h, 0, true);
    };
    auto verdict = [&]() {
        launch_assemble(h, active_groups(h), true, nullptr, 0, nullptr, true);
        check_and_compact();
        if (h->ld > 64) launch_assemble(h, active_groups(h), true, nullptr, 0, h->d_cflags + jg::CF_PERMUTE, true);
    };
    auto step = [&]() { const int rc = newton_step(h, active_groups(h), h->d_active); return rc ? fail(rc, h->eng.error) : 0; };
    int rc = h->gA.capture(h->stream, [&] { verdict(); return 0; });
    if (!rc) rc = h->gB.capture(h->stream, [&] { if (int rc = step()) return rc; verdict(); return 0; });
    if (!rc) rc = h->gBm.capture(h->stream, [&] {
        if (int rc = step()) return rc;
        launch_assemble(h, active_groups(h), false);
        check_and_compact();
        if (h->ld > 64) launch_assemble(h, active_groups(h), false, nullptr, 0, h->d_cflags + jg::CF_PERMUTE);
        return 0;
    });
    if (!rc) rc = h->gJ.capture(h->stream, [&] { launch_assemble(h, active_groups(h), true, nullptr, 0, nullptr, true); return 0; });
    if (rc) for (jg::Graph* g : {&h->gA, &h->gB, &h->gBm, &h->gJ}) g->reset();
    return rc;
}

void drop_iteration_graphs(jg_nr* h) {
    for (jg::Graph* g : {&h->gA, &h->gB, &h->gBm, &h->gJ, &h->gM}) g->reset();
    h->m_iters = 0;
}

int build_whole_graph(jg_nr* h, int k) {
    if (h->gM && h->m_iters == k) return 0;
    h->m_iters = 0;
    const int rc = h->gM.capture(h->stream, [&] {
        launch_assemble(h, active_groups(h), true, nullptr, 0, nullptr, true);
        launch_verdict64(h, false);
        for (int it = 1; it <= k; ++it) {
            if (int rc = newton_step(h, active_groups(h), h->d_active)) return fail(rc, h->eng.error);
            if (it < k) { launch_assemble(h, active_groups(h), true, nullptr, 0, nullptr, true); launch_verdict64(h, false); }
            else { launch_assemble(h, active_groups(h), false); launch_verdict64(h, true); }
        }
        return 0;
    });
    if (!rc) h->m_iters = k;
    return rc;
}

void drop_comp_graphs(jg_nr* h) { h->gA2.reset(); h->gC.reset(); }

void release_base(jg_nr_base* b) {
    if (!b) return;
    if (b->refs.fetch_sub(1) == 1) {
        hipSetDevice(b->device);
        b->cb.destroy();
        if (b->stream) hipStreamDestroy(b->stream);
        delete b;
    }
}

void detach_base(jg_nr* h) {
    if (!h->base) return;
    if (h->stream) hipStreamSynchronize(h->stream);
    drop_comp_graphs(h);
    h->release(&h->d_cw);
    release_base(h->base);
    h->base = nullptr;
    h->start_is_base = false;
}

int build_comp_graphs(jg_nr* h) {
    if (h->gC) return 0;
    const jg::CompBase& cb = h->base->cb;
    int rc = h->gA2.capture(h->stream, [&] {
        launch_assemble(h, active_groups(h), false);
        launch_check(h, 1, h->d_group);
        launch_compact(h, 0, true);
        if (h->ld > 64) launch_assemble(h, active_groups(h), false, nullptr, 0, h->d_cflags + jg::CF_PERMUTE);
        return 0;
    });
    if (!rc) rc = h->gC.capture(h->stream, [&] {
        jg::CompFixArgs fa{h->d_ppos, h->d_pdg, h->d_pdb, h->mp, cb.rowptr, cb.colm, cb.posrow, cb.rowtype, cb.v0, cb.th0, cb.y0, cb.Zc,
                           h->d_F, h->eng.status, h->d_active, h->ld, h->batch};
        if (h->mp > 0) jg::launch_comp_fix(fa, h->stream);
        jg::StateUpdate upd{h->d_va, h->d_vm, h->d_flags, h->d_active, -1.0};
        if (int rc = cb.solve(cb.split, h->stream, h->d_F, h->d_cw, h->d_inc, h->ld, h->batch, upd, active_groups(h))) return fail(rc, "the shared-factor sweep could not be captured");
        launch_assemble(h, active_groups(h), true, nullptr, 0, nullptr, true);
        launch_check(h, 1, h->d_group);
        launch_compact(h, 0, true);
        if (h->ld > 64) launch_assemble(h, active_groups(h), true, nullptr, 0, h->d_cflags + jg::CF_PERMUTE, true);
        return 0;
    });
    if (rc) drop_comp_graphs(h);
    return rc;
}

__global__ void k_cmp_injection(const double* p, const double* q, const double* p0, const double* q0, int n, int ld, int batch, int* count) {
    const int b = blockIdx.x * blockDim.x + threadIdx.x;
    if (b >= batch) return;
    int bad = 0;
    for (int i = blockIdx.y; i < n; i += gridDim.y) bad += (p[(size_t)i * ld + b] != p0[i]) || (q[(size_t)i * ld + b] != q0[i]);
    if (bad) atomicAdd(count, bad);
}

int comp_ready(jg_nr* h, bool& ready) {
    ready = false;
    if (!h->base || !h->first_mode || !h->start_is_base || h->refine || h->fast || h->lt_on) return 0;
    bool patched = false;
    for (unsigned char c : h->patch_state) { if (c == 2) return 0; patched |= c == 1; }
    if (patched) {
        if (!h->inj_checked) {
            NR_HIP(hipMemsetAsync(h->d_cmp, 0, sizeof(int), h->stream));
            hipLaunchKernelGGL(k_cmp_injection, dim3((h->batch + 255) / 256, 64), dim3(256), 0, h->stream, h->d_p, h->d_q, h->base->cb.p0, h->base->cb.q0, h->n, h->ld, h->batch, h->d_cmp);
            int bad = 0;
            NR_HIP(jg::sync_copy(&bad, h->d_cmp, sizeof(int), hipMemcpyDeviceToHost, h->stream));
            h->inj_checked = true; h->inj_equal = bad == 0;
        }
        if (!h->inj_equal) return 0;
    }
    if (int rc = build_comp_graphs(h)) return rc;
    ready = true;
    return 0;
}


int lt_rows(const jg_nr* h) { return (h->n + 31) / 32; }

void pack_types(const int8_t* type, int n, unsigned long long* words, int rows, size_t stride) {
    for (int r = 0; r < rows; ++r) {
        unsigned long long w = 0;
        for (int q = 0; q < 32 && r * 32 + q < n; ++q) w |= (unsigned long long)(type[r * 32 + q] & 3) << (2 * q);
        words[(size_t)r * stride] = w;
    }
}

int ensure_lane_types(jg_nr* h) {
    if (h->d_lt) return 0;
    const int rows = lt_rows(h);
    std::vector<unsigned long long> one(rows), all((size_t)rows * h->ld);
// ... 363 lines not shown
    for (int m = 0; m < h->mp; ++m) {
        const size_t off = (size_t)m * h->ld + scenario0;
        NR_HIP(jg::sync_copy(h->d_ppos + off, pos.data() + (size_t)m * wld, (size_t)count * sizeof(int), hipMemcpyHostToDevice, h->stream));
        NR_HIP(jg::sync_copy(h->d_pdg + off, g.data() + (size_t)m * wld, (size_t)count * sizeof(double), hipMemcpyHostToDevice, h->stream));
        NR_HIP(jg::sync_copy(h->d_pdb + off, b.data() + (size_t)m * wld, (size_t)count * sizeof(double), hipMemcpyHostToDevice, h->stream));
    }
    for (int64_t s = 0; s < count; ++s) h->patch_state[(size_t)(scenario0 + s)] = classify_patch(h, &allpos[(size_t)s * 8], h->mp);
    h->jac_valid = false;
    return 0;
}

int jg_nr_set_ybus(jg_nr* h, const double* y_reim, const double* yt_reim) {
    if (!h || !y_reim || !yt_reim) return fail(1, "jg_nr_set_ybus: bad argument");
    if (int rc = set_device(h)) return rc;
    std::vector<double> G(h->nnz), B(h->nnz);
    for (int p = 0; p < h->nnz; ++p) {
        G[p] = yt_reim[2 * p]; B[p] = yt_reim[2 * p + 1];
        if (y_reim[2 * (size_t)h->tperm[p]] != G[p] || y_reim[2 * (size_t)h->tperm[p] + 1] != B[p])
            return fail(4, "jg_nr_set_ybus: nodalMatrix and nodalMatrixTranspose disagree (stale model)");
    }
    NR_HIP(hipStreamSynchronize(h->stream));
    std::vector<double2> GBv(h->nnz);
    for (int p = 0; p < h->nnz; ++p) GBv[p] = double2{G[p], B[p]};
    NR_HIP(jg::sync_copy(h->d_GB, GBv.data(), GBv.size() * sizeof(double2), hipMemcpyHostToDevice, h->stream));
    h->jac_valid = false;
    detach_base(h);
    return 0;
}

int jg_nr_mismatch(jg_nr* h, double* max_p, double* max_q) {
    if (!h) return fail(1, "jg_nr_mismatch: bad argument");
    if (h->fast) return fail(1, "jg_nr_mismatch: this handle runs fast Newton-Raphson (its factor storage holds B', B''); use jg_nr_fast_mismatch");
    if (int rc = set_device(h)) return rc;
    launch_assemble(h);
    launch_check(h, 0);
    NR_HIP(hipGetLastError());
    NR_HIP(hipStreamSynchronize(h->stream));
    h->jac_valid = true;
    h->f_stale = false;
    if (max_p) NR_HIP(jg::sync_copy(max_p, h->d_normp, (size_t)h->batch * 8, hipMemcpyDeviceToHost, h->stream));
    if (max_q) NR_HIP(jg::sync_copy(max_q, h->d_normq, (size_t)h->batch * 8, hipMemcpyDeviceToHost, h->stream));
    return 0;
}

int jg_nr_solve(jg_nr* h) {
    if (!h) return fail(1, "jg_nr_solve: bad argument");
    if (h->fast) return fail(1, "jg_nr_solve: this handle runs fast Newton-Raphson; use jg_nr_fast_solve");
    if (int rc = set_device(h)) return rc;
    if (!h->jac_valid) launch_assemble(h);
    h->start_is_base = false;
    h->f_stale = false;
    NR_HIP(hipMemsetAsync(h->eng.status, 0, (size_t)h->ld * 4, h->stream));
    if (int rc = newton_step(h, jg::GroupSel{}, nullptr)) return fail(rc, h->eng.error);
    h->add_iter(h->d_iters);
    NR_HIP(hipGetLastError());
    NR_HIP(hipStreamSynchronize(h->stream));
    h->jac_valid = false;
    std::vector<int> st(h->ld);
    NR_HIP(jg::sync_copy(st.data(), h->eng.status, (size_t)h->ld * 4, hipMemcpyDeviceToHost, h->stream));
    for (int b = 0; b < h->batch; ++b) if (st[b] & 4) return fail(3, "jg_nr_solve: zero or non-finite pivot (singular Jacobian)");
    return 0;
}

int jg_nr_set_refine(jg_nr* h, int mode) {
    if (!h || mode < 0 || mode > 1) return fail(1, "jg_nr_set_refine: bad argument");
    if (h->fast) return fail(1, "jg_nr_set_refine: fast Newton-Raphson solves with constant matrices");
    if (mode && h->lt_on) return fail(1, "jg_nr_set_refine: scenarios have bus types of their own (jg_nr_set_bus_type / jg_nr_reactive_limit); the refinement residual reads the create-time types");
    if (int rc = set_device(h)) return rc;
    NR_HIP(hipStreamSynchronize(h->stream));
    if (mode && !h->d_R) {
        for (double** p : {&h->d_R, &h->d_inc2[0], &h->d_inc2[1]}) NR_HIP(h->alloc(p, (size_t)h->n * 2 * h->ld, true));
    }
    if ((mode != 0) != h->refine) {
        drop_iteration_graphs(h);
    }
    h->refine = mode != 0;
    h->eng.jordan = !h->refine && h->eng.plan->S.jordan && jg::knob("JORDAN", 1) != 0;
    return 0;
}

int jg_nr_set_shared(jg_nr* h, int mode) {
    if (!h || mode < 0 || mode > 1) return fail(1, "jg_nr_set_shared: bad argument");
    if (int rc = set_device(h)) return rc;
    NR_HIP(hipStreamSynchronize(h->stream));
    if ((mode != 0) != h->eng.shared) {
        drop_iteration_graphs(h);
    }
    h->eng.shared = mode != 0;
    return 0;
}

namespace {

int run_setup(jg_nr* h, int64_t max_iter, double tol, int lanes, bool keep_iters, int defer_at = 0) {
    if (int rc = build_graphs(h)) return rc;
    h->cmp.run_setup(h->stream, tol, (double)max_iter, (double)defer_at, lanes, keep_iters);
    NR_HIP(hipGetLastError());
    h->res_pinned = h->ld == 64;
    return 0;
}

int run_loop(jg_nr* h, int64_t max_iter, int defer_at) {
    const bool trace = jg::knob_set("TRACE");
    auto now_us = [] { return std::chrono::duration<double, std::micro>(std::chrono::steady_clock::now().time_since_epoch()).count(); };
    for (int64_t it = h->iter_graphs; it <= max_iter && *h->h_counter != 0; ++it) {
        if (defer_at > 0 && *h->h_counter <= defer_at) break;
        h->iter_graphs += 1;
        const bool guess_last = h->stop_hint > 0 && h->iter_graphs == h->stop_hint;
        const double tc = now_us();
        hipEvent_t e0 = nullptr, e1 = nullptr;
        if (trace) { hipEventCreate(&e0); hipEventCreate(&e1); hipEventRecord(e0, h->stream); }
        if (!trace) h->arm();
        NR_HIP((guess_last ? h->gBm : h->gB).launch(h->stream));
        const double tl = now_us();
        if (trace) hipEventRecord(e1, h->stream);
        NR_HIP(trace ? hipStreamSynchronize(h->stream) : h->wait());
        h->host_launch_us += tl - tc; h->host_wait_us += now_us() - tl; h->host_iters += 1;
        if (guess_last) {
            const bool stops = *h->h_counter == 0 || (defer_at > 0 && *h->h_counter <= defer_at) || it + 1 > max_iter;
            if (stops) h->last_guess_hit += 1;
            else { h->last_guess_miss += 1; NR_HIP(h->gJ.launch(h->stream)); }
        }
        if (trace) {
            float ms = 0.f; hipEventElapsedTime(&ms, e0, e1); fprintf(stderr, "[jg_nr_run] graph on the device: %.1f us\n", 1e3 * ms); hipEventDestroy(e0); hipEventDestroy(e1);
            int cf[4];
            jg::sync_copy(cf, h->d_cflags, sizeof(cf), hipMemcpyDeviceToHost, h->stream);
            fprintf(stderr, "[jg_nr_run] iteration %lld: %.1f us, %d scenarios still active, %d of %d lane groups in use%s%s\n", (long long)it + 1,
                    now_us() - tc, *h->h_counter, cf[jg::CF_GROUPS], h->ld / 64, cf[jg::CF_PERMUTE] ? " (compacted)" : "", guess_last ? " (verdict without a Jacobian)" : "");
        }
    }
    h->stop_hint = h->iter_graphs;
    return 0;
}

int run_start(jg_nr* h, int64_t max_iter) {
    bool comp = false;
    if (int rc = comp_ready(h, comp)) return rc;
    h->start_is_base = false;
    h->iter_graphs = 0;
    h->arm();
    NR_HIP((comp ? h->gA2 : h->gA).launch(h->stream));
    NR_HIP(h->wait());
    if (!comp) { h->first_full += 1; return 0; }
    h->first_comp += 1;
    if (max_iter < 1 || *h->h_counter == 0) {
        h->jac_valid = false;
        return 0;
    }
// ... 277 lines not shown
        NR_HIP(hipMemsetAsync(h->eng.status + lanes, 0, (size_t)(h->ld - lanes) * 4, h->stream));
        NR_HIP(hipMemsetD32Async((hipDeviceptr_t)(h->d_iters + lanes), (int)max_iter, (size_t)(h->ld - lanes), h->stream));
    }
    launch_compact(h, 0, true);
    launch_assemble(h, active_groups(h), true, nullptr, 0, nullptr, true);
    NR_HIP(hipStreamSynchronize(h->stream));
    h->iter_graphs = 0;
    if (int rc = run_loop(h, max_iter, 0)) return rc;
    h->paused = true;
    if (int rc = run_finish(h, nullptr, nullptr)) return rc;
    if (iters) NR_HIP(jg::sync_copy(iters, h->d_iters, (size_t)lanes * 4, hipMemcpyDeviceToHost, h->stream));
    if (status) NR_HIP(jg::sync_copy(status, h->d_status, (size_t)lanes * 4, hipMemcpyDeviceToHost, h->stream));
    return 0;
}

int jg_nr_pack_rows_device(jg_nr* h, double* dst_dev, int64_t lane0, int64_t count, const int32_t* rows) {
    if (!h || !dst_dev || !rows || lane0 < 0 || count < 0 || lane0 + count > h->batch || count > h->ld) return fail(1, "jg_nr_pack_rows_device: bad argument");
    if (count == 0) return 0;
    if (int rc = set_device(h)) return rc;
    NR_HIP(hipMemcpyAsync(h->d_itmp, rows, (size_t)count * 4, hipMemcpyHostToDevice, h->stream));
    hipLaunchKernelGGL(k_pack_rows, dim3((unsigned)std::min((h->n + 255) / 256, 64), (unsigned)count), dim3(256), 0, h->stream,
                       h->d_vm, h->d_va, h->d_iters, h->d_status, h->d_itmp, dst_dev, h->n, h->ld, (int)lane0, 2LL * h->n + 2);
    NR_HIP(hipGetLastError());
    NR_HIP(hipStreamSynchronize(h->stream));
    return 0;
}

static int get_scattered(jg_nr* h, const double* src, double* out) {
    std::vector<double> t((size_t)h->n * 2 * h->batch);
    if (int rc = h->get_rows2(src, t.data(), h->n)) return rc;
    for (int b = 0; b < h->batch; ++b) {
        const double* s = t.data() + (size_t)b * h->n * 2;
        double* d = out + (size_t)b * h->dimJ;
        for (int i = 0; i < h->n; ++i) {
            if (h->pvpq[i]) d[h->pvpq[i] - 1] = s[2 * i];
            if (h->pq[i]) d[h->pq[i] - 1] = s[2 * i + 1];
        }
    }
    return 0;
}

int jg_nr_get_mismatch(jg_nr* h, double* mism) {
    if (!h || !mism) return fail(1, "jg_nr_get_mismatch: bad argument");
    if (h->lt_on) return fail(1, "jg_nr_get_mismatch: scenarios have bus types of their own; the reference layout depends on the types");
    if (int rc = set_device(h)) return rc;
    if (h->f_stale) { launch_assemble(h, jg::GroupSel{}, false); NR_HIP(hipGetLastError()); h->f_stale = false; }
    NR_HIP(hipStreamSynchronize(h->stream));
    return get_scattered(h, h->d_F, mism);
}

int jg_nr_get_increment(jg_nr* h, double* incr) {
    if (!h || !incr) return fail(1, "jg_nr_get_increment: bad argument");
    if (h->lt_on) return fail(1, "jg_nr_get_increment: scenarios have bus types of their own; the reference layout depends on the types");
    if (int rc = set_device(h)) return rc;
    NR_HIP(hipStreamSynchronize(h->stream));
    return get_scattered(h, h->d_inc, incr);
}

int jg_nr_get_jacobian(jg_nr* h, double* nzval) {
    if (!h || !nzval) return fail(1, "jg_nr_get_jacobian: bad argument");
    if (h->lt_on) return fail(1, "jg_nr_get_jacobian: scenarios have bus types of their own; the reference layout depends on the types");
    if (h->fast) return fail(1, "jg_nr_get_jacobian: this handle runs fast Newton-Raphson: the factor storage holds the factorised B', B'', assembling the full Jacobian there would destroy them");
    if (int rc = set_device(h)) return rc;
    if (!h->jac_valid) { launch_assemble(h); h->jac_valid = true; }
    NR_HIP(hipStreamSynchronize(h->stream));
    std::vector<double> t((size_t)h->eng.plan->S.n_entries * 4 * h->ld);
    NR_HIP(jg::sync_copy(t.data(), h->eng.X, t.size() * 8, hipMemcpyDeviceToHost, h->stream));
    for (int b = 0; b < h->batch; ++b)
        for (int64_t k = 0; k < h->nnzJ; ++k) nzval[(size_t)b * h->nnzJ + k] = t[(((size_t)(h->jmap[k] >> 2) * 2 + ((h->jmap[k] >> 1) & 1)) * h->ld + b) * 2 + (h->jmap[k] & 1)];
    return 0;
}

int jg_nr_get_maps(jg_nr* h, int64_t* pq, int64_t* pvpq, int64_t* pcount, int64_t* jcolptr, int64_t* jrowval) {
    if (!h) return fail(1, "jg_nr_get_maps: bad argument");
    if (h->lt_on) return fail(1, "jg_nr_get_maps: scenarios have bus types of their own; the reference layout depends on the types");
    if (pq) std::memcpy(pq, h->pq.data(), h->pq.size() * 8);
    if (pvpq) std::memcpy(pvpq, h->pvpq.data(), h->pvpq.size() * 8);
    if (pcount) std::memcpy(pcount, h->pcount.data(), h->pcount.size() * 8);
    if (jcolptr) std::memcpy(jcolptr, h->jcolptr.data(), h->jcolptr.size() * 8);
    if (jrowval) std::memcpy(jrowval, h->jrowval.data(), h->jrowval.size() * 8);
    return 0;
}

int jg_nr_get_iteration(jg_nr* h, int32_t* iters) {
    if (!h || !iters) return fail(1, "jg_nr_get_iteration: bad argument");
    if (int rc = set_device(h)) return rc;
    NR_HIP(hipStreamSynchronize(h->stream));
    NR_HIP(jg::sync_copy(iters, h->d_iters, (size_t)h->batch * 4, hipMemcpyDeviceToHost, h->stream));
    return 0;
}

constexpr int FAST_MP = 4;
__global__ void k_fast_patch(double* X, const int* entry, const double* dp, const double* dq, int ld, int batch) {
    const int b = blockIdx.x * blockDim.x + threadIdx.x, m = blockIdx.y;
    if (b >= batch) return;
    const int e = entry[(size_t)m * batch + b];
    if (e < 0) return;
    double* x = X + ((size_t)e * 2 * ld + b) * 2;
    x[0] += dp[(size_t)m * batch + b];
    x[(size_t)ld * 2 + 1] += dq[(size_t)m * batch + b];
}

static int fast_refactor(jg_nr* h) {
    if (int rc = h->eng.set_shared_matrix(h->stream, h->fast_blk.data())) return fail(rc, h->eng.error);
    bool any = false;
    for (int e : h->fp_entry) any = any || e >= 0;
// ... 395 lines not shown
    for (int b = 0; b < h->batch; ++b) {
        if (count) count[b] = cnt[b];
        if (dead[b]) h->dead[b] = 1;
        else if (cnt[b] > 0) h->lt_set[b] = 1;
    }
    h->start_is_base = false;
    h->inj_checked = false;
    set_lane_types_on(h);
    return 0;
}

int jg_nr_adjust_angle(jg_nr* h, int64_t bus, double angle) {
    if (!h || bus < 1 || bus > h->n) return fail(1, "jg_nr_adjust_angle: bad argument (bus: 1-based index)");
    if (int rc = set_device(h)) return rc;
    if (!h->d_shift) NR_HIP(h->alloc(&h->d_shift, (size_t)h->ld));
    jg::adjust_angle_launch(h->d_shift, h->d_va, h->n, h->ld, h->batch, (int)bus - 1, angle, h->stream);
    NR_HIP(hipGetLastError());
    NR_HIP(hipStreamSynchronize(h->stream));
    h->jac_valid = false;
    h->start_is_base = false;
    return 0;
}

int jg_nr_time_kernel(jg_nr* h, int kernel, int reps, double* mean_ms) {
    if (!h || reps < 1 || !mean_ms || kernel < 0 || kernel > 5) return fail(1, "jg_nr_time_kernel: bad argument");
    if (kernel == 4 && (!h->base || !h->d_cw)) return fail(1, "jg_nr_time_kernel: kernel 4 (first iteration on the shared base factor) needs an attached base");
    if (h->fast && kernel < 2) return fail(1, "jg_nr_time_kernel: assembly / factorisation timing would overwrite the constant factor of a fast Newton-Raphson handle");
    if (int rc = set_device(h)) return rc;
    BranchArgs ba{};
    if (kernel == 3) {
        if (!h->d_bparam) return fail(1, "jg_nr_time_kernel: call jg_nr_set_branches first");
        const size_t one = (size_t)h->nb * h->ld * 2;
        if (int rc = post_staging(h, one * 7 * sizeof(double))) return rc;
        ba = BranchArgs{h->d_bfrom, h->d_bto, h->d_bstatus, h->d_bparam, h->d_vm, h->d_va, h->d_outage, h->d_post, h->d_post + one,
                        h->d_post + 2 * one, h->d_post + 3 * one, h->d_post + 4 * one, h->d_post + 5 * one, h->d_post + 6 * one,
                        h->nb, h->ld, h->batch};
    }
    hipEvent_t e0, e1;
    NR_HIP(hipEventCreate(&e0));
    NR_HIP(hipEventCreate(&e1));
    jg::StateUpdate none{};
    NR_HIP(hipStreamSynchronize(h->stream));
    {
        NR_HIP(hipEventRecord(e0, h->stream));
        for (int r = 0; r < reps; ++r) {
            if (kernel == 0) launch_assemble(h, jg::GroupSel{}, true, nullptr, 0, nullptr, true);
            else if (kernel == 1) { if (int rc = h->eng.factor(h->stream, nullptr, h->d_F, jg::GroupSel{}, h->eng.plan->S.prefactor != 0)) return fail(rc, h->eng.error); }
            else if (kernel == 3) hipLaunchKernelGGL(k_branch_quantities, dim3((h->nb + 15) / 16, h->ld / 64), dim3(64, 16), 0, h->stream, ba);
            else if (kernel == 4) {
                const jg::CompBase& cb = h->base->cb;
                jg::CompFixArgs fa{h->d_ppos, h->d_pdg, h->d_pdb, h->mp, cb.rowptr, cb.colm, cb.posrow, cb.rowtype, cb.v0, cb.th0, cb.y0, cb.Zc,
                                   h->d_F, h->eng.status, nullptr, h->ld, h->batch};
                if (h->mp > 0) jg::launch_comp_fix(fa, h->stream);
                if (int rc = cb.solve(cb.split, h->stream, h->d_F, h->d_cw, h->d_inc, h->ld, h->batch, none, jg::GroupSel{})) return fail(rc, "shared-factor sweep failed");
            }
            else if (kernel == 5) launch_assemble(h, jg::GroupSel{}, false);
            else { if (int rc = h->eng.backsolve(h->stream, h->d_inc, none, jg::GroupSel{})) return fail(rc, h->eng.error); }
        }
        NR_HIP(hipEventRecord(e1, h->stream));
    }
    NR_HIP(hipEventSynchronize(e1));
    float ms = 0.f;
    NR_HIP(hipEventElapsedTime(&ms, e0, e1));
    hipEventDestroy(e0); hipEventDestroy(e1);
    if (kernel <= 1) h->jac_valid = false;
    *mean_ms = (double)ms / reps;
    return 0;
}

}
```

### juliagrid.jl_amd/csrc/jg_plan_api.cpp

```cpp
#include <cstring>
#include <string>
#include <vector>

#include "../../include/jgrid.h"
#include "jg_symbolic.hpp"

struct jg_plan {
    jg::BlockSymbolic S;
};

extern "C" {

int jg_plan_create(jg_plan** out, int64_t n, const int32_t* rowptr, const int32_t* col, int64_t policy) {
    if (!out || !rowptr || !col || n < 1) return 1;
    jg_plan* p = new jg_plan();
    if (jg::analyze((int)n, rowptr, col, (long long)policy, p->S)) { delete p; return 1; }
    *out = p;
    return 0;
}

void jg_plan_destroy(jg_plan* p) { delete p; }

int64_t jg_plan_export(jg_plan* p, int which, int32_t* out, int64_t cap) {
    if (!p) return -1;
    if (which == 68 || which == 69) jg::build_selected_inverse(p->S);
    const jg::BlockSymbolic& S = p->S;
    std::vector<int> tmp;
    const std::vector<int>* v = nullptr;
    switch (which) {
        case 0: v = &S.perm; break;   case 1: v = &S.e_row; break;  case 2: v = &S.e_col; break;
        case 3: v = &S.e_src; break;  case 4: v = &S.t_ptr; break;  case 5: v = &S.t_a; break;
        case 6: v = &S.t_b; break;    case 7: v = &S.e_level; break; case 8: v = &S.e_diag; break;
        case 9: v = &S.diag; break;   case 10: v = &S.l_ptr; break; case 11: v = &S.l_ent; break;
        case 12: v = &S.l_col; break; case 13: v = &S.u_ptr; break; case 14: v = &S.u_ent; break;
        case 15: v = &S.u_col; break;  case 16: v = &S.t_d; break;  case 17: v = &S.y_level; break;
        case 18: v = &S.bwd_level; break;
        case 60: tmp.assign((const int*)S.fact_seg.data(), (const int*)S.fact_seg.data() + S.fact_seg.size() * 8); v = &tmp; break;
        case 61: tmp.assign((const int*)S.fact_rec.data(), (const int*)S.fact_rec.data() + S.fact_rec.size() * 16); v = &tmp; break;
        case 62: tmp.assign((const int*)S.bwd_seg.data(), (const int*)S.bwd_seg.data() + S.bwd_seg.size() * 8); v = &tmp; break;
        case 63: tmp.assign((const int*)S.bwd_rec.data(), (const int*)S.bwd_rec.data() + S.bwd_rec.size() * 16); v = &tmp; break;
        case 64: v = &S.src_entry; break;
        case 65: v = &S.bwd_chain; break;
        case 66: tmp.assign((const int*)S.fwd_seg.data(), (const int*)S.fwd_seg.data() + S.fwd_seg.size() * 8); v = &tmp; break;
        case 67: tmp.assign((const int*)S.fwd_rec.data(), (const int*)S.fwd_rec.data() + S.fwd_rec.size() * 16); v = &tmp; break;
        case 19: v = &S.chain_level; break;
        case 68: tmp.assign((const int*)S.sel_seg.data(), (const int*)S.sel_seg.data() + S.sel_seg.size() * 8); v = &tmp; break;
        case 69: tmp.assign((const int*)S.sel_rec.data(), (const int*)S.sel_rec.data() + S.sel_rec.size() * 16); v = &tmp; break;
        case 70: tmp.assign((const int*)S.top_task.data(), (const int*)S.top_task.data() + S.top_task.size() * 16); v = &tmp; break;
        case 71: v = &S.top_data; break;
        case 72: tmp.assign((const int*)S.top_launch.data(), (const int*)S.top_launch.data() + S.top_launch.size() * 8); v = &tmp; break;
        case 78: v = &S.top_wgmap; break;
        case 73: v = &S.top_task_of; break;
        case 74: tmp = {S.top_level, (int)(S.top_stack & 0x7fffffff), (int)(S.top_terms & 0x7fffffff), (int)S.top_stack_cls[0], (int)S.top_stack_cls[1], (int)S.top_stack_cls[2], S.jordan, S.n_jordan,
                        S.fact_tasks, S.task_rounds, (int)S.n_staged, (int)S.n_direct_terms}; v = &tmp; break;
        case 79: tmp.assign((const int*)S.bwdj_seg.data(), (const int*)S.bwdj_seg.data() + S.bwdj_seg.size() * 8); v = &tmp; break;
        case 80: tmp.assign((const int*)S.bwdj_rec.data(), (const int*)S.bwdj_rec.data() + S.bwdj_rec.size() * 16); v = &tmp; break;
        case 81: tmp.assign((const int*)S.f_rec.data(), (const int*)S.f_rec.data() + S.f_rec.size() * 16); v = &tmp; break;
        case 82: v = &S.f1_first; break;
        case 83: v = &S.f1_wg; break;
        case 84: v = &S.f2_first; break;
        case 85: tmp = {S.single_fact_ok ? 1 : 0, S.n_f1_wg, jg::SINGLE_FACT_LEVELS, jg::SINGLE_FACT_ITEMS}; v = &tmp; break;
        case 90: case 91: case 92: case 93: case 94: case 95: case 96: case 97: case 98: case 99: case 100: {
            jg::SingleTables T;
            jg::build_single_tables(S, T);
            switch (which) {
                case 90: tmp = {T.ok ? 1 : 0, T.n_top, T.n_top_levels, T.n_bottom, T.n_wg, T.b_levels, jg::SINGLE_BOTTOM_ROWS, T.flat_ok ? 1 : 0, T.max_level_terms, T.max_level_rows}; break;
                case 91: tmp = T.t_row; break;  case 92: tmp = T.t_ptr; break;  case 93: tmp = T.t_term; break;  case 94: tmp = T.t_level; break;
                case 95: tmp = T.b_wg; break;   case 96: tmp = T.b_row; break;  case 97: tmp = T.b_term; break;
                case 98: tmp = T.t_jb; break;   case 99: tmp = T.t_cslot; break; default: tmp = T.t_toff; break;
            }
            v = &tmp; break;
        }
        case 101: tmp.assign(S.top_dead.begin(), S.top_dead.end()); v = &tmp; break;
        case 102: tmp = {S.top_dead_ok, (int)(S.top_dead_blocks & 0x7fffffff), (int)(S.top_store_blocks & 0x7fffffff)}; v = &tmp; break;
        case 75: tmp.assign(S.pre_pivot.begin(), S.pre_pivot.end()); v = &tmp; break;
        case 76: tmp.assign((const int*)S.pre_seg.data(), (const int*)S.pre_seg.data() + S.pre_seg.size() * 8); v = &tmp; break;
        case 77: tmp.assign((const int*)S.pre_rec.data(), (const int*)S.pre_rec.data() + S.pre_rec.size() * 16); v = &tmp; break;
        default: return -1;
    }
    if (!out) return (int64_t)v->size();
    if ((int64_t)v->size() > cap) return -1;
    if (!v->empty()) std::memcpy(out, v->data(), v->size() * sizeof(int));
    return (int64_t)v->size();
}

int64_t jg_plan_comp_export(jg_plan* p, int64_t top_cap, int which, int32_t* out, int64_t cap) {
    if (!p || which < 0 || which > 5) return -1;
    jg::CompTables T;
    jg::build_comp_tables(p->S, (int)top_cap, T);
    std::vector<int> tmp;
    switch (which) {
        case 0: tmp = {T.n_top, T.split, T.n_fwd_levels, T.n_bwd_levels}; break;
        case 1: tmp = T.top; break;
        case 2: tmp.assign((const int*)T.fwd_seg.data(), (const int*)T.fwd_seg.data() + T.fwd_seg.size() * 8); break;
        case 3: tmp.assign((const int*)T.fwd_rec.data(), (const int*)T.fwd_rec.data() + T.fwd_rec.size() * 16); break;
        case 4: tmp.assign((const int*)T.bwd_seg.data(), (const int*)T.bwd_seg.data() + T.bwd_seg.size() * 8); break;
        default: tmp.assign((const int*)T.bwd_rec.data(), (const int*)T.bwd_rec.data() + T.bwd_rec.size() * 16); break;
    }
    if (!out) return (int64_t)tmp.size();
    if ((int64_t)tmp.size() > cap) return -1;
    if (!tmp.empty()) std::memcpy(out, tmp.data(), tmp.size() * sizeof(int));
    return (int64_t)tmp.size();
}

}
```

### juliagrid.jl_amd/csrc/jg_symbolic.cpp

```cpp
#include "jg_symbolic.hpp"

#include <algorithm>
#include <atomic>
#include <chrono>
#include <type_traits>
#include <iterator>
#include <queue>
#include <system_error>
#include <thread>
#include <cstdio>
#include <cstring>
#include <string>
#include <cstdlib>
#include <numeric>

namespace jg {

int knob(const char* name, int unset) {
    static const char* const known[] = {"TRACE", "PLAN_CACHE", "POLL", "PLAN_THREADS", "PLAN_TIMING", "HOST_TIMING",
                                        "TOP_PW", "TOP_FUSE", "TOP_SYM", "JORDAN", "CHAIN_SMALL", "NO_PREFACTOR", "LANES_INPLACE", "TOP_LEVEL", "ROW_TASKS", "ORDER_CHECK", "TOP_PROFILE", "SINGLE", "SWEEP_ONLY"};
    bool ok = false;
    for (const char* k : known) ok = ok || std::strcmp(k, name) == 0;
    if (!ok) return unset;
    const std::string var = std::string("JG_") + name;
    const char* e = getenv(var.c_str());
    return e ? atoi(e) : unset;
}


void build_tables(BlockSymbolic& S);
constexpr int NO_TOP_LEVEL = 0x7fffffff;
void build_top(BlockSymbolic& S, int top_level, int soft_cap, int struct_min, int mid_mmin, int mid_strict);

namespace {

bool elimination_order(int n, std::vector<std::vector<int>>&& adj0, std::vector<int>& order,
                       std::vector<std::vector<int>>& strct) {
    bool exact = true;
    std::vector<std::vector<int>> adj = std::move(adj0);
    std::vector<char> done(n, 0);
    std::vector<int> hv(n, 0), mark(n, -1), seen(n, -1), hits(n, 0);
    std::vector<long long> cur(n, 0), fillv(n, 0);
    int stamp = 0;
    auto fill_of = [&](int v) -> long long {
        const std::vector<int>& nb = adj[v];
        const long long d = (long long)nb.size();
        ++stamp;
        for (int a : nb) mark[a] = stamp;
        long long present = 0;
        for (int a : nb) {
            const std::vector<int>& aa = adj[a];
            long long c = 0;
            for (size_t x = 0; x < aa.size(); ++x) c += mark[aa[x]] == stamp;
            present += c;
        }
        return d * (d - 1) / 2 - present / 2;
    };
    const long long wf = 20, wh = 0, wd = 0, wq = 1;
    auto key_of = [&](int v) -> long long {
        const long long d = (long long)adj[v].size(), h = hv[v];
        return ((wf * fillv[v] + wh * h + wd * d + wq * h * h) << 20) | std::min<long long>(d, (1 << 20) - 1);
    };
    auto key = [&](int v) -> long long { fillv[v] = fill_of(v); return key_of(v); };
    std::vector<int> hp(n), hpos(n);
    int hn = 0;
    auto before = [&](int a, int b) { return cur[a] < cur[b] || (cur[a] == cur[b] && a < b); };
    auto sift_up = [&](int i) {
        const int v = hp[i];
        while (i > 0) { const int p = (i - 1) >> 2; if (!before(v, hp[p])) break; hp[i] = hp[p]; hpos[hp[i]] = i; i = p; }
        hp[i] = v; hpos[v] = i;
    };
    auto sift_down = [&](int i) {
        const int v = hp[i];
// ... 957 lines not shown
    }
    std::vector<int> count(maxlev + 2, 0);
    for (int r = 0; r < n; ++r) count[flev[r]]++;
    int split = maxlev;
    if (top_cap >= 0) {
        int above = 0;
        while (split > 1 && above + count[split] <= top_cap) { above += count[split]; --split; }
    }
    out.split = split;
    out.tpos.assign(n, -1);
    for (int r = 0; r < n; ++r) if (flev[r] > split) { out.tpos[r] = (int)out.top.size(); out.top.push_back(r); }
    out.n_top = (int)out.top.size();
    const std::vector<int>& tpos = out.tpos;
    {
        std::vector<int> level(n, 0), work(n, 0);
        for (int r = 0; r < n; ++r) {
            if (tpos[r] < 0) { level[r] = flev[r]; work[r] = S.l_ptr[r + 1] - S.l_ptr[r]; continue; }
            int l = 1, w = 0;
            for (int p = S.l_ptr[r]; p < S.l_ptr[r + 1]; ++p) if (tpos[S.l_col[p]] < 0) { l = std::max(l, flev[S.l_col[p]] + 1); ++w; }
            level[r] = l; work[r] = w;
        }
        build_replay(level, work, COMP_T, out.fwd_seg, out.fwd_rec, out.n_fwd_levels, [&](int k, int sub, int wpi, int rpw, Rec* r) {
            for (int j = 0; j < rpw; ++j) { r[j].w[0] = tpos[k] < 0 ? k : n + tpos[k]; r[j].w[1] = S.perm[k]; r[j].w[2] = -1; r[j].w[3] = 0; }
            int q = 0, seen = 0;
            for (int p = S.l_ptr[k]; p < S.l_ptr[k + 1]; ++p) {
                if (tpos[k] >= 0 && tpos[S.l_col[p]] >= 0) continue;
                if (seen++ % wpi != sub) continue;
                Rec& x = r[q / COMP_T];
                const int s = 4 + 2 * (q % COMP_T);
                x.w[s] = S.l_ent[p]; x.w[s + 1] = S.l_col[p];
                x.w[3]++; ++q;
            }
        }, NoExtra(), 0, 8);
    }
    {
        std::vector<int> level(n, 0), work(n, 0);
        for (int r = n - 1; r >= 0; --r) {
            if (tpos[r] >= 0) continue;
            int l = 1;
            for (int p = S.u_ptr[r]; p < S.u_ptr[r + 1]; ++p) if (tpos[S.u_col[p]] < 0) l = std::max(l, level[S.u_col[p]] + 1);
            level[r] = l; work[r] = S.u_ptr[r + 1] - S.u_ptr[r];
        }
        build_replay(level, work, COMP_T, out.bwd_seg, out.bwd_rec, out.n_bwd_levels, [&](int k, int sub, int wpi, int rpw, Rec* r) {
            for (int j = 0; j < rpw; ++j) { r[j].w[0] = k; r[j].w[1] = S.perm[k]; r[j].w[2] = S.diag[k]; r[j].w[3] = 0; }
            int q = 0;
            for (int p = S.u_ptr[k] + sub; p < S.u_ptr[k + 1]; p += wpi, ++q) {
                Rec& x = r[q / COMP_T];
                const int s = 4 + 2 * (q % COMP_T);
                x.w[s] = S.u_ent[p]; x.w[s + 1] = S.u_col[p];
                x.w[3]++;
            }
        }, NoExtra(), 0, 8);
    }
}

void build_single_tables(const BlockSymbolic& S, SingleTables& T) {
    T = SingleTables();
    const int n = S.n;
    if (!S.jordan || S.top_task.empty() || S.symmetric) return;
    std::vector<int> jrow(n, -1), jroot(n, -1), tlev(n, 0);
    int max_tl = 0;
    for (const Rec& h : S.top_task) max_tl = std::max(max_tl, h.w[10]);
    for (const Rec& h : S.top_task) {
        const int* piv = S.top_data.data() + h.w[3] + h.w[6];
        for (int q = 0; q < h.w[0]; ++q) { jrow[piv[q]] = h.w[14] >= 0 ? h.w[14] + q * h.w[1] : 0; jroot[piv[q]] = h.w[2]; tlev[piv[q]] = max_tl - h.w[10]; }
    }
    std::vector<int> rows;
    for (int k = 0; k < n; ++k) if (jroot[k] >= 0) rows.push_back(k);
    std::stable_sort(rows.begin(), rows.end(), [&](int a, int b) { return tlev[a] < tlev[b]; });
    T.n_top = (int)rows.size();
    T.n_top_levels = max_tl;
    std::vector<int> slot(n, -1);
    for (int i = 0; i < T.n_top; ++i) slot[rows[i]] = i;
    T.t_level.assign(max_tl + 1, 0);
    for (int k : rows) T.t_level[tlev[k] + 1]++;
    for (int l = 0; l < max_tl; ++l) T.t_level[l + 1] += T.t_level[l];
    std::vector<int> slist(n, -1);
    for (int k : rows) {
        const int root = jroot[k], e = S.u_ptr[root + 1] - S.u_ptr[root];
        if (slist[root] < 0) {
            slist[root] = (int)T.t_term.size();
            for (int t = 0; t < e; ++t) {
                const int c = S.u_col[S.u_ptr[root] + t];
                if (slot[c] < 0 || tlev[c] >= tlev[k]) return;
                T.t_term.push_back(slot[c]);
            }
        }
        T.t_row.push_back(k); T.t_row.push_back(S.perm[k]); T.t_row.push_back(S.diag[k]); T.t_row.push_back(e);
        T.t_ptr.push_back(e > 0 ? jrow[k] - S.n_entries : 0); T.t_ptr.push_back(slist[root]);
    }
    if (T.t_term.empty()) T.t_term.push_back(0);
    {
        T.flat_ok = true;
        T.t_jb.assign(2 * (size_t)max_tl, 0);
        T.t_cslot.assign((size_t)std::max(S.n_jordan, 1), 0);
        long long covered = 0;
        for (int l = 0; l < max_tl; ++l) {
            T.max_level_rows = std::max(T.max_level_rows, T.t_level[l + 1] - T.t_level[l]);
            int first = -1, terms = 0;
            for (int i = T.t_level[l]; i < T.t_level[l + 1]; ++i) {
                const int e = T.t_row[4 * i + 3], jb = T.t_ptr[2 * i], sl = T.t_ptr[2 * i + 1];
                T.t_toff.push_back(terms);
                if (e == 0) continue;
                if (first < 0) first = jb;
                if (jb != first + terms || jb + e > S.n_jordan) { T.flat_ok = false; break; }
                for (int t = 0; t < e; ++t) T.t_cslot[jb + t] = T.t_term[sl + t];
// ... 220 lines not shown
    S.u_ptr.assign(n + 1, 0);
    for (int r = 0; r < n; ++r) { S.l_ptr[r + 1] = S.l_ptr[r] + lcount[r]; S.u_ptr[r + 1] = S.u_ptr[r] + (int)strct[r].size(); }
    S.l_ent.assign(S.l_ptr[n], 0); S.l_col.assign(S.l_ptr[n], 0);
    S.u_ent.assign(S.u_ptr[n], 0); S.u_col.assign(S.u_ptr[n], 0);
    for (int r = 0; r < n; ++r) {
        int lp = S.l_ptr[r], up = S.u_ptr[r];
        for (int e = S.row_ptr[r]; e < S.row_ptr[r + 1]; ++e) {
            int c = S.e_col[e];
            if (c < r) { S.l_ent[lp] = e; S.l_col[lp++] = c; }
            else if (c > r) { S.u_ent[up] = e; S.u_col[up++] = c; }
        }
    }
    S.y_level.assign(n, S.prefactor ? 0 : 1);
    S.bwd_level.assign(n, 1);
    for (int r = 0; r < n; ++r)
        for (int p = S.l_ptr[r]; p < S.l_ptr[r + 1]; ++p) {
            const int c = S.l_col[p];
            S.y_level[r] = std::max(S.y_level[r], 1 + std::max(S.y_level[c], std::max(S.e_level[S.l_ent[p]], S.e_level[S.diag[c]])));
        }
    for (int r = n - 1; r >= 0; --r)
        for (int p = S.u_ptr[r]; p < S.u_ptr[r + 1]; ++p) S.bwd_level[r] = std::max(S.bwd_level[r], S.bwd_level[S.u_col[p]] + 1);

    {
        int top_level = (policy >> 8) & 0xff, soft = (policy >> 16) & 0xff;
        if (knob_set("TOP_LEVEL")) top_level = knob("TOP_LEVEL", top_level);
        if (top_level == 0) {
            int narrow = ((policy >> 24) & 0x7f) * 8;
            if (narrow == 0) narrow = TOP_NARROW;
            if (narrow == 127 * 8) narrow = 0x7fffffff;
            int nlev = 0;
            for (int e = 0; e < S.n_entries; ++e) nlev = std::max(nlev, S.e_level[e]);
            for (int r = 0; r < n; ++r) nlev = std::max(nlev, S.y_level[r]);
            int chains = (policy >> 4) & 0xf;
            if (chains >= 13) chains = chains == 13 ? 18 : (chains == 14 ? 24 : 36);
            if (S.want_single && chains == 0) chains = 150;
            std::vector<int> cnt(nlev + 2, 0), piv(nlev + 2, 0);
            for (int e = 0; e < S.n_entries; ++e) if (!(S.symmetric && S.e_row[e] > S.e_col[e])) cnt[S.e_level[e]]++;
            for (int r = 0; r < n; ++r) { cnt[S.y_level[r]]++; piv[S.e_level[S.diag[r]]]++; }
            top_level = nlev + 1;
            const int level_min = TOP_LEVEL_MIN - (S.prefactor ? 1 : 0);
            while (top_level > level_min && cnt[top_level - 1] <= narrow && (chains == 0 || piv[top_level - 1] <= chains)) --top_level;
            if (top_level > nlev - 2) top_level = NO_TOP_LEVEL;
        } else if (top_level >= 255) top_level = NO_TOP_LEVEL;
        if (soft <= 0) soft = TOP_FRONT_SOFT;
        int struct_min = 0, mid_mmin = 0, mid_strict = (int)((policy64 >> 48) & 1);
        if (const int mid = (int)((policy64 >> 32) & 0xff)) { struct_min = mid; mid_mmin = (int)((policy64 >> 40) & 0xff); if (!mid_mmin) mid_mmin = 6; }
        lap("fill pattern, terms, levels");
        build_top(S, top_level, std::min(soft, TOP_FRONT_MAX), struct_min, mid_mmin, mid_strict);
        lap("top tasks");
    }
    if (S.n_entries + S.n_jordan >= (1 << 24)) S.fact_tasks = 0;
    build_tables(S);
    mark_sweep_dead(S);
    lap("replay tables");
    return 0;
}

void mark_sweep_dead(BlockSymbolic& S) {
    S.top_dead.assign((size_t)S.n_entries, 0);
    S.top_dead_ok = 0; S.top_dead_blocks = 0; S.top_store_blocks = 0;
    if (!S.jordan || S.symmetric || S.top_task.empty()) return;
    std::vector<int> seen((size_t)S.n_entries, 0);
    long long half = 0;
    for (const Rec& h : S.top_task) {
        const int m = h.w[0], e = h.w[1], f = m + e, fprime = h.w[11];
        const int* emap = S.top_data.data() + h.w[3];
        for (int r = 0; r < f; ++r)
            for (int c = 0; c < f; ++c) {
                const int cd = emap[(size_t)r * fprime + c];
                if (r < m && c >= m) continue;
                if (cd < 0 || ((cd >> 28) & 4)) continue;
                S.top_dead[cd & 0x0fffffff] = 1; seen[cd & 0x0fffffff]++;
            }
        half += 2LL * m  + 2LL * m * e  + m  + 2LL * e * (e + 1) ;
    }
    long long cand = 0;
    bool struck = false;
    for (int en = 0; en < S.n_entries; ++en) if (S.top_dead[en]) { ++cand; if (seen[en] != 1) struck = true; }
    auto read = [&](int en) { if (en >= 0 && en < S.n_entries && S.top_dead[en]) { S.top_dead[en] = 0; struck = true; } };
    auto scan_fact = [&](const std::vector<Rec>& recs) {
        for (const Rec& r : recs) {
            if (r.w[0] < 0) continue;
            for (int t = 0; t < r.w[3] && t < FACT_T; ++t) {
                read(r.w[4 + 3 * t] & 0x3fffffff); read(r.w[5 + 3 * t]);
                if (r.w[0] != 3) read(r.w[6 + 3 * t]);
            }
        }
    };
    auto scan_tasks = [&](const std::vector<Rec>& recs) {
        for (const Rec& r : recs) {
            for (int u = 0; u < ((r.w[3] >> 8) & 0xff) && u < TASK_STAGE; ++u) { read(r.w[10 + 3 * u] & 0xffffff); read(r.w[11 + 3 * u]); }
            const int kind = r.w[0] & TK_KIND, nt = r.w[3] & 0xff;
            if (kind == 7) continue;
            for (int t = 0; t < nt; ++t) {
                if (r.w[0] & TK_DIRECT) {
                    if (t >= TASK_DIRECT_T) break;
                    read(r.w[4 + 3 * t] & 0x3fffffff); read(r.w[5 + 3 * t]);
                    if (kind != 3) read(r.w[6 + 3 * t]);
                } else if (t < TASK_T && kind != 3) read(r.w[4 + t] & 0xffffff);
            }
        }
    };
    if (S.fact_tasks) scan_tasks(S.fact_rec); else scan_fact(S.fact_rec);
    scan_fact(S.pre_rec);
    for (const Segment& sg : S.bwdj_seg) {
        if (sg.wpi <= 0) {
            for (int x = 0; x < sg.nchunks; ++x) {
                const Rec& r = S.bwdj_rec[(size_t)sg.rec_base + x];
                const int nb = r.w[0], nE = r.w[1];
                const int* d = S.bwd_chain.data() + r.w[2];
                for (int p = 0; p < nb; ++p) read(d[3 * p + 2]);
                const int* u = d + 3 * nb + nE;
                for (int q = 0; q < nb * nE + nb * nb; ++q) read(u[q]);
            }
            continue;
        }
        const size_t nrec = (size_t)sg.nchunks * 16 * sg.rpw;
        for (size_t x = 0; x < nrec; ++x) {
            const Rec& r = S.bwdj_rec[(size_t)sg.rec_base + x];
            if (r.w[0] < 0) continue;
            read(r.w[2]);
            for (int t = 0; t < r.w[3] && t < BWD_T; ++t) read(r.w[4 + 2 * t]);
        }
    }
    S.top_dead_ok = struck ? 0 : 1;
    for (int en = 0; en < S.n_entries; ++en) if (S.top_dead[en]) S.top_dead_blocks++;
    S.top_store_blocks = half + 2 * cand;
    S.top_dead_blocks *= 2;
}

}
```

### juliagrid.jl_amd/csrc/jg_symbolic.hpp

```cpp
#pragma once
#include <cstdint>
#include <vector>

namespace jg {

int knob(const char* name, int unset);
inline bool knob_set(const char* name) { return knob(name, -2147483647) != -2147483647; }

struct Segment {
    int rec_base;
    int nchunks;
    int wpi;
    int rpw;
    int level;
    int last;
    int items;
    int pad;
};
constexpr int FACT_T = 4;
constexpr int FACT_WAVES = 8;
constexpr int BWD_T = 6;
constexpr int TASK_WAVES = 8, TASK_SLOTS = 30, TASK_T = 6, TASK_STAGE = 2, TASK_DIRECT_T = 2;
constexpr int TK_KIND = 7, TK_FIRST = 8, TK_LAST = 16, TK_BAR = 32, TK_SIDE = 64, TK_DIRECT = 128;
constexpr int CHAIN_MAX_ROWS = 32, CHAIN_MAX_EXT = 72, CHAIN_SMALL_ROWS = 8;
// ... 13 lines not shown
    std::vector<int> e_src;
    std::vector<int> e_diag;
    std::vector<int> diag;
    std::vector<int> t_ptr, t_a, t_d, t_b;
    std::vector<int> e_level;
    std::vector<int> l_ptr, l_ent, l_col;
    std::vector<int> u_ptr, u_ent, u_col;
    std::vector<int> y_level, bwd_level;
    long long n_terms = 0;
    long long n_sched_terms = 0;
    int inplace = 0;
    int symmetric = 0;
    int prefactor = 0;
    int top_split = 0;
    std::vector<char> pre_pivot;
    std::vector<Segment> pre_seg; std::vector<Rec> pre_rec; int n_pre_levels = 0;
    std::vector<int> src_entry;
    std::vector<Segment> fact_seg, bwd_seg, fwd_seg;
    std::vector<Rec> fact_rec, bwd_rec, fwd_rec;
    int fact_tasks = 0;
    int task_rounds = 0;
    long long n_staged = 0;
    long long n_direct_terms = 0;
    int jordan = 0;
    int n_jordan = 0;
    std::vector<Segment> bwdj_seg;
    std::vector<Rec> bwdj_rec;
    int n_bwdj_levels = 0;
    std::vector<int> bwd_chain;
    std::vector<int> chain_level;
    int n_fact_levels = 0, n_bwd_levels = 0, n_fwd_levels = 0;
    std::vector<Segment> sel_seg;
    std::vector<Rec> sel_rec;
    int n_sel_levels = 0;
    int top_level = 0;
    int want_single = 0;
    bool single_fact_ok = false;
    std::vector<Rec> f_rec;
    std::vector<int> f1_first, f1_wg, f2_first;
    int n_f1_wg = 0;
    int top_mmin = 8;
    std::vector<int> top_task_of;
    std::vector<Rec> top_task;
    std::vector<int> top_data;
    std::vector<TopLaunch> top_launch;
    std::vector<int> top_wgmap;
    long long top_stack = 0;
    long long top_stack_cls[3] = {0, 0, 0};
    long long top_terms = 0;
    std::vector<char> top_dead;
    int top_dead_ok = 0;
    long long top_dead_blocks = 0;
    long long top_store_blocks = 0;
};

constexpr int COMP_T = 6;
struct CompTables {
    int n_top = 0, split = 0;
    std::vector<int> top;
    std::vector<int> tpos;
    std::vector<Segment> fwd_seg, bwd_seg;
    std::vector<Rec> fwd_rec, bwd_rec;
    int n_fwd_levels = 0, n_bwd_levels = 0;
};
void build_comp_tables(const BlockSymbolic& S, int top_cap, CompTables& out);

constexpr int SINGLE_FACT_LEVELS = 8;
constexpr int SINGLE_FACT_ITEMS = 192;
constexpr int SINGLE_BOTTOM_ROWS = 256;
constexpr int SINGLE_BOTTOM_FILL = 128;
struct SingleTables {
    bool ok = false;
    int n_top = 0, n_top_levels = 0;
    std::vector<int> t_row, t_ptr, t_term, t_level;
    bool flat_ok = false;
    std::vector<int> t_jb, t_cslot, t_toff;
    int max_level_terms = 0, max_level_rows = 0;
    int n_bottom = 0, n_wg = 0, b_levels = 0;
    std::vector<int> b_wg;
    std::vector<int> b_row, b_term;
};
void build_single_tables(const BlockSymbolic& S, SingleTables& out);

int analyze(int n, const int* rowptr, const int* col, long long policy, BlockSymbolic& out);
void build_selected_inverse(BlockSymbolic& S);
void mark_sweep_dead(BlockSymbolic& S);
int entry_of(const BlockSymbolic& S, int r, int c);

}
```

Baseline: 401,200.

## Skip dead backward-sweep stores and optional bus-order increment output

Adds a symbolic pass that marks rows whose backward-sweep solution is never read by a later record, tags them with a high bit in the device tables, and skips their W stores in the batched sweep kernels. Also adds a handle option to drop the bus-order increment output, which the contingency pipeline switches off. Both changes cut global memory writes in the triangular sweeps. The cost is extra masking of packed indices, plus a new API state where get_increment is unavailable.

```diff
diff --git a/include/jgrid.h b/include/jgrid.h
--- a/include/jgrid.h
+++ b/include/jgrid.h
@@ -41,6 +41,7 @@
 int jg_nr_solve(jg_nr* h);
 int jg_nr_set_refine(jg_nr* h, int mode);
 int jg_nr_set_shared(jg_nr* h, int mode);
+int jg_nr_set_keep_increment(jg_nr* h, int mode);
 int jg_nr_run(jg_nr* h, int64_t max_iter, double tol, int32_t* iters, int32_t* status);
 int jg_nr_run_defer(jg_nr* h, int64_t max_iter, double tol, int64_t defer_at, int32_t* n_left);
 int jg_nr_move_lanes(jg_nr* dst, int64_t dst_lane0, jg_nr* src, int32_t* home, int32_t* count);
diff --git a/juliagrid.jl_amd/_lib.py b/juliagrid.jl_amd/_lib.py
--- a/juliagrid.jl_amd/_lib.py
+++ b/juliagrid.jl_amd/_lib.py
@@ -56,6 +56,7 @@
         "jg_nr_solve": [VP],
         "jg_nr_set_refine": [VP, C.c_int],
         "jg_nr_set_shared": [VP, C.c_int],
+        "jg_nr_set_keep_increment": [VP, C.c_int],
         "jg_nr_run": [VP, C.c_int64, C.c_double, I32P, I32P],
         "jg_nr_run_defer": [VP, C.c_int64, C.c_double, C.c_int64, C.POINTER(C.c_int32)],
         "jg_nr_move_lanes": [VP, C.c_int64, VP, I32P, C.POINTER(C.c_int32)],
diff --git a/juliagrid.jl_amd/contingency.py b/juliagrid.jl_amd/contingency.py
--- a/juliagrid.jl_amd/contingency.py
+++ b/juliagrid.jl_amd/contingency.py
@@ -263,6 +263,8 @@
         if len(self.handles) + len(self.pools) > 1:
             for an in self.handles + [p.handle for p in self.pools]:
                 _lib.check(_lib.lib().jg_nr_set_shared(an._h, 1))
+        for an in self.handles + [p.handle for p in self.pools]:
+            _lib.check(_lib.lib().jg_nr_set_keep_increment(an._h, 0))
         if start is not None:
             self.setStart(*start)
         else:
diff --git a/juliagrid.jl_amd/csrc/jg_comp.hip b/juliagrid.jl_amd/csrc/jg_comp.hip
--- a/juliagrid.jl_amd/csrc/jg_comp.hip
+++ b/juliagrid.jl_amd/csrc/jg_comp.hip
@@ -34,6 +34,7 @@
     GroupSel sel; StateUpdate upd;
     int ld, seg_begin, lanes;
     int s0_base, s0_nchunks, s0_wpi, s0_rpw;
+    int dead_ok;
 };
 
 __device__ __forceinline__ void csweep_record(const CSweepArgs& a, const RecS& r, size_t ld, unsigned off, double& a0, double& a1) {
@@ -74,7 +75,7 @@
     const size_t ri = (size_t)base + ((size_t)bx * 8 + wave) * rpw;
     const RecS first = load_rec(a.rec, ri);
     const int sub = wave & (wpi - 1);
-    const int k = first[0], src = first[1], dg = first[2];
+    const int k = first[0], src = first[1], dgw = first[2], dg = dgw & BWD_ENTRY_MASK;
     double a0 = 0.0, a1 = 0.0;
     int fl = 0; bool act = true; double va = 0.0, vm = 0.0;
     if (k >= 0) {
@@ -105,9 +106,9 @@
     if (wpi > 1) __syncthreads();
     if (k >= 0 && sub == 0) {
         for (int w = 1; w < wpi; ++w) { const double2 p = ((const double2*)red)[(size_t)(wave + w) * 64 + lane]; a0 += p.x; a1 += p.y; }
-        store_vec(a.W, (size_t)k, b, ld, a0, a1);
+        if (!(BWD && a.dead_ok && ((dgw >> BWD_DEAD_BIT) & 1))) store_vec(a.W, (size_t)k, b, ld, a0, a1);
         if (BWD) {
-            if (!a.upd.va || act) store_vec(a.out, (size_t)src, b, ld, a0, a1);
+            if (a.out && (!a.upd.va || act)) store_vec(a.out, (size_t)src, b, ld, a0, a1);
             if (a.upd.va) {
                 if (act && (fl & 1)) a.upd.va[(size_t)src * ld + b] = va + a.upd.sign * a0;
                 if (act && (fl & 2)) a.upd.vm[(size_t)src * ld + b] = vm + a.upd.sign * a1;
@@ -122,6 +123,7 @@
     const int* piv; const int* bus;
     double* W; double* out; GroupSel sel; StateUpdate upd;
     int ld, lanes, n, n_top, n_rb;
+    int dead_ok;
 };
 typedef double d4v __attribute__((ext_vector_type(4)));
 __global__ __launch_bounds__(64 * CTOP_WAVES) void k_ctop(CTopArgs a) {
@@ -178,9 +180,9 @@
 #pragma unroll
         for (int w = 0; w < CTOP_WAVES; ++w) x += part[w][j][r][lane];
         if (t >= a.n_top) continue;
-        const int k = a.piv[t], bus = a.bus[t];
-        a.W[((size_t)k * ld + b) * 2 + c] = x;
-        if (!a.upd.va || act) a.out[((size_t)bus * ld + b) * 2 + c] = x;
+        const int kw = a.piv[t], k = kw & BWD_ENTRY_MASK, bus = a.bus[t];
+        if (!(a.dead_ok && ((kw >> BWD_DEAD_BIT) & 1))) a.W[((size_t)k * ld + b) * 2 + c] = x;
+        if (a.out && (!a.upd.va || act)) a.out[((size_t)bus * ld + b) * 2 + c] = x;
         if (a.upd.va && act) {
             const int fl = (int)a.upd.flags[bus];
             double* st = c == 0 ? a.upd.va : a.upd.vm;
@@ -230,7 +232,7 @@
 __global__ void k_take_sinv(const double* W, const int* piv, double* Sinv, int n_ks, int n_top, int ld, int col0, int count) {
     const int b = blockIdx.x * blockDim.x + threadIdx.x, i = blockIdx.y;
     if (b >= count || i >= n_top) return;
-    const double2 x = *(const double2*)(W + ((size_t)piv[i] * ld + b) * 2);
+    const double2 x = *(const double2*)(W + ((size_t)(piv[i] & BWD_ENTRY_MASK) * ld + b) * 2);
     const int kc = col0 + b, ks = kc >> 2, kq = kc & 3;
     for (int c = 0; c < 2; ++c) {
         const int r = 2 * i + c, rb = r >> 4, rr = r & 15;
@@ -358,8 +360,12 @@
     build_comp_tables(S, top_cap, T);
     std::vector<int> bus(T.top.size());
     for (size_t i = 0; i < T.top.size(); ++i) bus[i] = S.perm[T.top[i]];
-    if (upload(&fwd_rec, T.fwd_rec, err, st) || upload(&fwd_seg, T.fwd_seg, err, st) || upload(&bwd_rec, T.bwd_rec, err, st) || upload(&bwd_seg, T.bwd_seg, err, st) ||
-        upload(&top_piv, T.top, err, st) || upload(&top_bus, bus, err, st)) return 2;
+    std::vector<Rec> bwd_dev = T.bwd_rec;
+    std::vector<int> top_dev = T.top;
+    for (Rec& r : bwd_dev) if (r.w[0] >= 0 && T.dead[r.w[0]]) r.w[2] |= 1 << BWD_DEAD_BIT;
+    for (int& k : top_dev) if (T.dead[k]) k |= 1 << BWD_DEAD_BIT;
+    if (upload(&fwd_rec, T.fwd_rec, err, st) || upload(&fwd_seg, T.fwd_seg, err, st) || upload(&bwd_rec, bwd_dev, err, st) || upload(&bwd_seg, T.bwd_seg, err, st) ||
+        upload(&top_piv, top_dev, err, st) || upload(&top_bus, bus, err, st)) return 2;
     auto launches = [](const std::vector<Segment>& segs, std::vector<DevLaunch>& out) {
         out.clear();
         size_t s = 0;
@@ -384,8 +390,8 @@
     fwd_rec = bwd_rec = nullptr; fwd_seg = bwd_seg = nullptr; top_piv = top_bus = nullptr;
 }
 
-int CompBase::solve(const CompSweep& sw, hipStream_t st, const double* rhs, double* Wc, double* out, int ld, int lanes, const StateUpdate& upd, const GroupSel& sel) const {
-    CSweepArgs a{sw.fwd_rec, sw.fwd_seg, Mc, rhs, Wc, out, sel, StateUpdate{}, ld, 0, lanes, 0, 0, 1, 1};
+int CompBase::solve(const CompSweep& sw, hipStream_t st, const double* rhs, double* Wc, double* out, int ld, int lanes, const StateUpdate& upd, const GroupSel& sel, bool dead_ok) const {
+    CSweepArgs a{sw.fwd_rec, sw.fwd_seg, Mc, rhs, Wc, out, sel, StateUpdate{}, ld, 0, lanes, 0, 0, 1, 1, dead_ok ? 1 : 0};
     for (const DevLaunch& L : sw.fwd) {
         a.seg_begin = L.seg_begin;
         { const Segment& g = sw.T.fwd_seg[L.seg_begin]; a.s0_base = g.rec_base; a.s0_nchunks = g.nchunks; a.s0_wpi = g.wpi; a.s0_rpw = g.rpw; }
@@ -393,7 +399,7 @@
     }
     if (sw.T.n_top > 0) {
         const int n_rb = (2 * sw.T.n_top + 15) / 16;
-        CTopArgs t{Sinv, lds, sw.top_piv, sw.top_bus, Wc, out, sel, upd, ld, lanes, n, sw.T.n_top, n_rb};
+        CTopArgs t{Sinv, lds, sw.top_piv, sw.top_bus, Wc, out, sel, upd, ld, lanes, n, sw.T.n_top, n_rb, dead_ok ? 1 : 0};
         hipLaunchKernelGGL(k_ctop, dim3(grid_blocks(ld / 64, n_rb)), dim3(64, CTOP_WAVES), 0, st, t);
     }
     a.rec = sw.bwd_rec; a.seg = sw.bwd_seg; a.upd = upd;
diff --git a/juliagrid.jl_amd/csrc/jg_comp.hpp b/juliagrid.jl_amd/csrc/jg_comp.hpp
--- a/juliagrid.jl_amd/csrc/jg_comp.hpp
+++ b/juliagrid.jl_amd/csrc/jg_comp.hpp
@@ -25,7 +25,7 @@
 
     int create(const BlockSymbolic& S, const double* Xsrc, int ldx, int top_cap, hipStream_t st);
     void destroy();
-    int solve(const CompSweep& sw, hipStream_t st, const double* rhs, double* Wc, double* out, int ld, int lanes, const StateUpdate& upd, const GroupSel& sel) const;
+    int solve(const CompSweep& sw, hipStream_t st, const double* rhs, double* Wc, double* out, int ld, int lanes, const StateUpdate& upd, const GroupSel& sel, bool dead_ok = false) const;
     size_t scratch_rows(const CompSweep& sw) const { return (size_t)n + (size_t)((sw.T.n_top + 7) & ~7); }
 };
 
diff --git a/juliagrid.jl_amd/csrc/jg_engine.hip b/juliagrid.jl_amd/csrc/jg_engine.hip
--- a/juliagrid.jl_amd/csrc/jg_engine.hip
+++ b/juliagrid.jl_amd/csrc/jg_engine.hip
@@ -26,6 +26,7 @@
     int ld, seg_begin;
     int lanes;
     int s0_base, s0_nchunks, s0_wpi, s0_rpw;
+    int dead_ok;
 };
 
 
@@ -181,11 +182,11 @@
     }
     return p;
 }
-__device__ __forceinline__ double2 bwd_finish(const BwdArgs& a, const Blk& d, double y0, double y1, int k, int bus, size_t b, size_t ld, const UpdPre& p) {
+__device__ __forceinline__ double2 bwd_finish(const BwdArgs& a, const Blk& d, double y0, double y1, int k, int bus, int dgw, size_t b, size_t ld, const UpdPre& p) {
     double x0, x1;
     dsolve(d, y0, y1, x0, x1);
-    store_vec(a.W, (size_t)k, b, ld, x0, x1);
-    if (!a.upd.va || p.act) store_vec(a.out, (size_t)bus, b, ld, x0, x1);
+    if (!(a.dead_ok && ((dgw >> BWD_DEAD_BIT) & 1))) store_vec(a.W, (size_t)k, b, ld, x0, x1);
+    if (a.out && (!a.upd.va || p.act)) store_vec(a.out, (size_t)bus, b, ld, x0, x1);
     if (a.upd.va) {
         if (p.act && (p.fl & 1)) a.upd.va[(size_t)bus * ld + b] = p.va + a.upd.sign * x0;
         if (p.act && (p.fl & 2)) a.upd.vm[(size_t)bus * ld + b] = p.vm + a.upd.sign * x1;
@@ -245,7 +246,7 @@
     Blk mb[CHAIN_PF][2], db[CHAIN_PF];
     auto request = [&](int c, Blk (&m)[2], Blk& d) {
         if (c < 0) return;
-        if (wave == (c & 15)) d = load_blk(a.X, (size_t)rows[3 * c + 2], b, ld);
+        if (wave == (c & 15)) d = load_blk(a.X, (size_t)(rows[3 * c + 2] & BWD_ENTRY_MASK), b, ld);
 #pragma unroll
         for (int i = 0; i < 2; ++i) { const int p = wave + 16 * i; if (p < c) m[i] = load_blk(a.X, (size_t)uin[p * nb + c], b, ld); }
     };
@@ -259,7 +260,7 @@
                 double2* slot = xc + (c & 1) * 64;
                 if (wave == (c & 15)) {
                     const double2 y = acc[c * 64 + lane];
-                    slot[lane] = bwd_finish(a, db[s], y.x, y.y, rows[3 * c], rows[3 * c + 1], b, ld, c < 16 ? up0 : up1);
+                    slot[lane] = bwd_finish(a, db[s], y.x, y.y, rows[3 * c], rows[3 * c + 1], rows[3 * c + 2], b, ld, c < 16 ? up0 : up1);
                 }
                 __syncthreads();
                 const double2 x = slot[lane];
@@ -294,14 +295,15 @@
     UpdPre up{0, false, 0.0, 0.0};
     double y0 = 0.0, y1 = 0.0;
     Blk d{0.0, 0.0, 0.0, 0.0};
-    int k = 0, bus = 0;
+    int k = 0, bus = 0, dgw = 0;
     Blk mb[CHAIN_PF];
     auto request = [&](int c, Blk& m) { if (owner && c > p) m = load_blk(a.X, (size_t)uin[p * nb + c], b, ld); };
     if (owner) {
         k = rows[3 * p]; bus = rows[3 * p + 1];
         up = upd_prefetch(a, bus, b, ld);
         const double2 y = load_vec(a.W, (size_t)k, b, ld); y0 = y.x; y1 = y.y;
-        d = load_blk(a.X, (size_t)rows[3 * p + 2], b, ld);
+        dgw = rows[3 * p + 2];
+        d = load_blk(a.X, (size_t)(dgw & BWD_ENTRY_MASK), b, ld);
     }
 #pragma unroll
     for (int s = 0; s < CHAIN_PF; ++s) request(nb - 1 - s, mb[s]);
@@ -332,7 +334,7 @@
             const int c = c0 - s;
             if (c >= 0) {
                 double2* slot = xc + (c & 1) * 64;
-                if (owner && p == c) slot[lane] = bwd_finish(a, d, y0, y1, k, bus, b, ld, up);
+                if (owner && p == c) slot[lane] = bwd_finish(a, d, y0, y1, k, bus, dgw, b, ld, up);
                 if (c > 0) {
                     __syncthreads();
                     if (owner && p < c) {
@@ -350,7 +352,7 @@
 __device__ __forceinline__ void bwd_chunk(const BwdArgs& a, double* red, const RecS& first, size_t rec_index, int rpw, int wpi,
                                           int wave, int lane, size_t b, size_t ld) {
     const int sub = wave & (wpi - 1);
-    const int k = rec_word(first, 0), bus = rec_word(first, 1), dg = rec_word(first, 2);
+    const int k = rec_word(first, 0), bus = rec_word(first, 1), dgw = rec_word(first, 2), dg = dgw & BWD_ENTRY_MASK;
     double y0 = 0.0, y1 = 0.0;
     Blk d{0.0, 0.0, 0.0, 0.0};
     UpdPre up{0, false, 0.0, 0.0};
@@ -373,7 +375,7 @@
     if (wpi > 1) __syncthreads();
     if (k >= 0 && sub == 0) {
         for (int w = 1; w < wpi; ++w) { const double2 p = ((const double2*)red)[(size_t)(wave + w) * 64 + lane]; y0 += p.x; y1 += p.y; }
-        bwd_finish(a, d, y0, y1, k, bus, b, ld, up);
+        bwd_finish(a, d, y0, y1, k, bus, dgw, b, ld, up);
     }
     if (wpi > 1) __syncthreads();
 }
@@ -1864,10 +1866,24 @@
     const double tu0 = std::chrono::duration<double, std::milli>(std::chrono::steady_clock::now().time_since_epoch()).count();
     std::vector<int> prow(n, 0);
     for (int k = 0; k < n; ++k) if (S.prefactor && S.pre_pivot[k]) prow[S.perm[k]] = k + 1;
+    std::vector<Rec> bwdj_dev = S.bwdj_rec;
+    std::vector<int> chain_dev = S.bwd_chain;
+    if (S.bwd_dead_ok)
+        for (const Segment& sg : S.bwdj_seg) {
+            if (sg.wpi <= 0) {
+                for (int x = 0; x < sg.nchunks; ++x) {
+                    const Rec& r = S.bwdj_rec[(size_t)sg.rec_base + x];
+                    for (int q = 0; q < r.w[0]; ++q) { int* row = chain_dev.data() + r.w[2] + 3 * q; if (S.bwd_dead[row[0]]) row[2] |= 1 << BWD_DEAD_BIT; }
+                }
+                continue;
+            }
+            const size_t nrec = (size_t)sg.nchunks * 16 * sg.rpw;
+            for (size_t x = 0; x < nrec; ++x) { Rec& r = bwdj_dev[(size_t)sg.rec_base + x]; if (r.w[0] >= 0 && S.bwd_dead[r.w[0]]) r.w[2] |= 1 << BWD_DEAD_BIT; }
+        }
     if (upload(&p->pre_rec, S.pre_rec, error, st) || upload(&p->pre_seg, S.pre_seg, error, st) || upload(&p->pre_row, prow, error, st) ||
         upload(&p->fact_rec, S.fact_rec, error, st) || upload(&p->bwd_rec, S.bwd_rec, error, st) || upload(&p->fact_seg, S.fact_seg, error, st) ||
-        upload(&p->bwd_seg, S.bwd_seg, error, st) || upload(&p->bwd_chain, S.bwd_chain, error, st) ||
-        (S.jordan && (upload(&p->bwdj_rec, S.bwdj_rec, error, st) || upload(&p->bwdj_seg, S.bwdj_seg, error, st))) ||
+        upload(&p->bwd_seg, S.bwd_seg, error, st) || upload(&p->bwd_chain, chain_dev, error, st) ||
+        (S.jordan && (upload(&p->bwdj_rec, bwdj_dev, error, st) || upload(&p->bwdj_seg, S.bwdj_seg, error, st))) ||
         upload(&p->fwd_rec, S.fwd_rec, error, st) || upload(&p->fwd_seg, S.fwd_seg, error, st) ||
         (S.single_fact_ok && (upload(&p->f1_rec, S.f_rec, error, st) || upload(&p->f1_wg, S.f1_wg, error, st))) ||
         (!S.top_launch.empty() && (upload(&p->top_task, S.top_task, error, st) || upload(&p->top_data, S.top_data, error, st) || upload(&p->top_wgmap, S.top_wgmap, error, st)))) {
@@ -2154,6 +2170,7 @@
 int Engine::backsolve(hipStream_t st, double* out, const StateUpdate& upd, const GroupSel& sel) {
     if (single_bwd && jordan) {
         const SingleTables& T = plan->single;
+        if (!out) { error = "backsolve: the single-instance sweep always stores the bus-order solution (out = nullptr is for the batched level kernels)"; return 1; }
         Bwd1Args s{plan->s1_t_row, plan->s1_t_ptr, plan->s1_t_term, plan->s1_t_level, plan->s1_b_wg, plan->s1_b_row, plan->s1_b_term, X, jc, W, out, sel, upd, ld, T.n_top_levels, T.n_wg, T.n_top,
                    plan->s1_t_jb, plan->s1_t_cslot, plan->s1_t_toff, T.max_level_terms};
         const int flat_env = knob("SINGLE", 1);
@@ -2163,7 +2180,8 @@
         JG_HIP(hipGetLastError());
         return 0;
     }
-    BwdArgs a{jordan ? plan->bwdj_rec : bwd_rec, jordan ? plan->bwdj_seg : bwd_seg, bwd_chain, X, W, out, sel, upd, ld, 0, lanes > 0 ? lanes : ld, 0, 0, 1, 1};
+    const int dead_ok = sweep_only && jordan && plan->S.jordan && plan->S.bwd_dead_ok && !Zs && knob("SWEEP_DEAD", 1) != 0 ? 1 : 0;
+    BwdArgs a{jordan ? plan->bwdj_rec : bwd_rec, jordan ? plan->bwdj_seg : bwd_seg, bwd_chain, X, W, out, sel, upd, ld, 0, lanes > 0 ? lanes : ld, 0, 0, 1, 1, dead_ok};
     const std::vector<Segment>& segs = jordan ? plan->S.bwdj_seg : plan->S.bwd_seg;
     for (const DevLaunch& L : (jordan ? bwdj : bwd)) {
         a.seg_begin = L.seg_begin;
diff --git a/juliagrid.jl_amd/csrc/jg_nr.hip b/juliagrid.jl_amd/csrc/jg_nr.hip
--- a/juliagrid.jl_amd/csrc/jg_nr.hip
+++ b/juliagrid.jl_amd/csrc/jg_nr.hip
@@ -518,6 +518,8 @@
     int* d_lid = nullptr; int* d_dest = nullptr; int* d_cflags = nullptr; int* d_itmp = nullptr; int* d_glist = nullptr;
     jg::Compaction cmp{};
     bool refine = false;
+    bool keep_inc = true;
+    bool inc_fresh = true;
     bool fast = false;
     std::vector<double> fast_blk;
     std::vector<int> fp_entry; std::vector<double> fp_dp, fp_dq;
@@ -596,6 +598,9 @@
     return (b < 0 || joined) ? 1 : 2;
 }
 
+double* inc_out(jg_nr* h) { return h->keep_inc || h->eng.single_bwd ? h->d_inc : nullptr; }
+bool comp_dead_ok(jg_nr* h) { return h->eng.sweep_only && !h->refine && jg::knob("SWEEP_DEAD", 1) != 0; }
+
 jg::GroupSel active_groups(jg_nr* h) { return jg::GroupSel{nullptr, h->d_glist, h->d_cflags + jg::CF_LIST}; }
 
 template <class F> void with_mp(int mp, F&& f) {
@@ -714,7 +719,7 @@
 void launch_compact(jg_nr* h, int restore, bool report = false) {
     std::vector<jg::LaneRows> rows{{h->d_vm, h->n, 1}, {h->d_va, h->n, 1}, {h->d_p, h->n, 1}, {h->d_q, h->n, 1}};
     if (h->mp > 0) { rows.push_back({h->d_pdg, h->mp, 1}); rows.push_back({h->d_pdb, h->mp, 1}); }
-    rows.push_back({h->d_inc, h->n, 2});
+    if (h->keep_inc) rows.push_back({h->d_inc, h->n, 2});
     if (h->lt_on) rows.push_back({(double*)h->d_lt, (h->n + 31) / 32, 1});
     h->cmp.launch_compact(h->stream, restore, report, rows);
 }
@@ -723,7 +728,7 @@
     if (int rc = h->eng.factor(h->stream, nullptr, h->d_F, sel, h->level0_done)) return rc;
     if (!h->refine) {
         jg::StateUpdate upd{h->d_va, h->d_vm, h->lt_on ? h->d_flags_all : h->d_flags, active, -1.0};
-        return h->eng.backsolve(h->stream, h->d_inc, upd, sel);
+        return h->eng.backsolve(h->stream, inc_out(h), upd, sel);
     }
     jg::StateUpdate none{};
     if (int rc = h->eng.backsolve(h->stream, h->d_inc2[1], none, sel)) return rc;
@@ -824,7 +829,7 @@
                            h->d_F, h->eng.status, h->d_active, h->ld, h->batch};
         if (h->mp > 0) jg::launch_comp_fix(fa, h->stream);
         jg::StateUpdate upd{h->d_va, h->d_vm, h->d_flags, h->d_active, -1.0};
-        if (int rc = cb.solve(cb.split, h->stream, h->d_F, h->d_cw, h->d_inc, h->ld, h->batch, upd, active_groups(h))) return fail(rc, "the shared-factor sweep could not be captured");
+        if (int rc = cb.solve(cb.split, h->stream, h->d_F, h->d_cw, inc_out(h), h->ld, h->batch, upd, active_groups(h), comp_dead_ok(h))) return fail(rc, "the shared-factor sweep could not be captured");
         launch_assemble(h, active_groups(h), true, nullptr, 0, nullptr, true);
         launch_check(h, 1, h->d_group);
         launch_compact(h, 0, true);
@@ -1294,6 +1299,7 @@
     h->f_stale = false;
     NR_HIP(hipMemsetAsync(h->eng.status, 0, (size_t)h->ld * 4, h->stream));
     if (int rc = newton_step(h, jg::GroupSel{}, nullptr)) return fail(rc, h->eng.error);
+    if (h->keep_inc) h->inc_fresh = true;
     h->add_iter(h->d_iters);
     NR_HIP(hipGetLastError());
     NR_HIP(hipStreamSynchronize(h->stream));
@@ -1307,6 +1313,7 @@
 int jg_nr_set_refine(jg_nr* h, int mode) {
     if (!h || mode < 0 || mode > 1) return fail(1, "jg_nr_set_refine: bad argument");
     if (h->fast) return fail(1, "jg_nr_set_refine: fast Newton-Raphson solves with constant matrices");
+    if (mode && !h->keep_inc && h->paused) return fail(1, "jg_nr_set_refine: the handle is paused (jg_nr_run_defer) and keeps no increment (jg_nr_set_keep_increment); finish it first");
     if (mode && h->lt_on) return fail(1, "jg_nr_set_refine: scenarios have bus types of their own (jg_nr_set_bus_type / jg_nr_reactive_limit); the refinement residual reads the create-time types");
     if (int rc = set_device(h)) return rc;
     NR_HIP(hipStreamSynchronize(h->stream));
@@ -1316,11 +1323,29 @@
     if ((mode != 0) != h->refine) {
         drop_iteration_graphs(h);
     }
+    if (mode && !h->keep_inc) {
+        if (int rc = jg_nr_set_keep_increment(h, 1)) return rc;
+    }
     h->refine = mode != 0;
     h->eng.jordan = !h->refine && h->eng.plan->S.jordan && jg::knob("JORDAN", 1) != 0;
     return 0;
 }
 
+int jg_nr_set_keep_increment(jg_nr* h, int mode) {
+    if (!h || mode < 0 || mode > 1) return fail(1, "jg_nr_set_keep_increment: bad argument");
+    if (mode == 0 && h->refine) return fail(1, "jg_nr_set_keep_increment: iterative refinement (jg_nr_set_refine) writes the increment; switch it off first");
+    if (h->paused) return fail(1, "jg_nr_set_keep_increment: the handle is paused (jg_nr_run_defer); finish it first");
+    if ((mode != 0) == h->keep_inc) return 0;
+    if (int rc = set_device(h)) return rc;
+    NR_HIP(hipStreamSynchronize(h->stream));
+    drop_iteration_graphs(h);
+    drop_comp_graphs(h);
+    if (mode) NR_HIP(jg::sync_fill(h->d_inc, 0, (size_t)h->n * 2 * h->ld * 8, h->stream));
+    h->keep_inc = mode != 0;
+    h->inc_fresh = false;
+    return 0;
+}
+
 int jg_nr_set_shared(jg_nr* h, int mode) {
     if (!h || mode < 0 || mode > 1) return fail(1, "jg_nr_set_shared: bad argument");
     if (int rc = set_device(h)) return rc;
@@ -1336,6 +1361,7 @@
 
 int run_setup(jg_nr* h, int64_t max_iter, double tol, int lanes, bool keep_iters, int defer_at = 0) {
     if (int rc = build_graphs(h)) return rc;
+    if (h->keep_inc) h->inc_fresh = true;
     h->cmp.run_setup(h->stream, tol, (double)max_iter, (double)defer_at, lanes, keep_iters);
     NR_HIP(hipGetLastError());
     h->res_pinned = h->ld == 64;
@@ -1719,6 +1745,8 @@
 int jg_nr_get_increment(jg_nr* h, double* incr) {
     if (!h || !incr) return fail(1, "jg_nr_get_increment: bad argument");
     if (h->lt_on) return fail(1, "jg_nr_get_increment: scenarios have bus types of their own; the reference layout depends on the types");
+    if (!h->keep_inc) return fail(1, "jg_nr_get_increment: this handle keeps no bus-order increment (jg_nr_set_keep_increment(h, 0)); switch it on and run again");
+    if (!h->inc_fresh) return fail(1, "jg_nr_get_increment: jg_nr_set_keep_increment was switched on after the last run; the increment is there after the next one");
     if (int rc = set_device(h)) return rc;
     NR_HIP(hipStreamSynchronize(h->stream));
     return get_scattered(h, h->d_inc, incr);
@@ -2220,10 +2248,10 @@
                 jg::CompFixArgs fa{h->d_ppos, h->d_pdg, h->d_pdb, h->mp, cb.rowptr, cb.colm, cb.posrow, cb.rowtype, cb.v0, cb.th0, cb.y0, cb.Zc,
                                    h->d_F, h->eng.status, nullptr, h->ld, h->batch};
                 if (h->mp > 0) jg::launch_comp_fix(fa, h->stream);
-                if (int rc = cb.solve(cb.split, h->stream, h->d_F, h->d_cw, h->d_inc, h->ld, h->batch, none, jg::GroupSel{})) return fail(rc, "shared-factor sweep failed");
+                if (int rc = cb.solve(cb.split, h->stream, h->d_F, h->d_cw, inc_out(h), h->ld, h->batch, none, jg::GroupSel{}, comp_dead_ok(h))) return fail(rc, "shared-factor sweep failed");
             }
             else if (kernel == 5) launch_assemble(h, jg::GroupSel{}, false);
-            else { if (int rc = h->eng.backsolve(h->stream, h->d_inc, none, jg::GroupSel{})) return fail(rc, h->eng.error); }
+            else { if (int rc = h->eng.backsolve(h->stream, inc_out(h), none, jg::GroupSel{})) return fail(rc, h->eng.error); }
         }
         NR_HIP(hipEventRecord(e1, h->stream));
     }
diff --git a/juliagrid.jl_amd/csrc/jg_plan_api.cpp b/juliagrid.jl_amd/csrc/jg_plan_api.cpp
--- a/juliagrid.jl_amd/csrc/jg_plan_api.cpp
+++ b/juliagrid.jl_amd/csrc/jg_plan_api.cpp
@@ -73,6 +73,8 @@
         }
         case 101: tmp.assign(S.top_dead.begin(), S.top_dead.end()); v = &tmp; break;
         case 102: tmp = {S.top_dead_ok, (int)(S.top_dead_blocks & 0x7fffffff), (int)(S.top_store_blocks & 0x7fffffff)}; v = &tmp; break;
+        case 103: tmp.assign(S.bwd_dead.begin(), S.bwd_dead.end()); v = &tmp; break;
+        case 104: tmp = {S.bwd_dead_ok, S.bwd_dead_rows}; v = &tmp; break;
         case 75: tmp.assign(S.pre_pivot.begin(), S.pre_pivot.end()); v = &tmp; break;
         case 76: tmp.assign((const int*)S.pre_seg.data(), (const int*)S.pre_seg.data() + S.pre_seg.size() * 8); v = &tmp; break;
         case 77: tmp.assign((const int*)S.pre_rec.data(), (const int*)S.pre_rec.data() + S.pre_rec.size() * 16); v = &tmp; break;
@@ -85,7 +87,7 @@
 }
 
 int64_t jg_plan_comp_export(jg_plan* p, int64_t top_cap, int which, int32_t* out, int64_t cap) {
-    if (!p || which < 0 || which > 5) return -1;
+    if (!p || which < 0 || which > 7) return -1;
     jg::CompTables T;
     jg::build_comp_tables(p->S, (int)top_cap, T);
     std::vector<int> tmp;
@@ -95,6 +97,8 @@
         case 2: tmp.assign((const int*)T.fwd_seg.data(), (const int*)T.fwd_seg.data() + T.fwd_seg.size() * 8); break;
         case 3: tmp.assign((const int*)T.fwd_rec.data(), (const int*)T.fwd_rec.data() + T.fwd_rec.size() * 16); break;
         case 4: tmp.assign((const int*)T.bwd_seg.data(), (const int*)T.bwd_seg.data() + T.bwd_seg.size() * 8); break;
+        case 6: tmp.assign(T.dead.begin(), T.dead.end()); break;
+        case 7: tmp = {T.n_dead, T.n_dead_top}; break;
         default: tmp.assign((const int*)T.bwd_rec.data(), (const int*)T.bwd_rec.data() + T.bwd_rec.size() * 16); break;
     }
     if (!out) return (int64_t)tmp.size();
diff --git a/juliagrid.jl_amd/csrc/jg_symbolic.cpp b/juliagrid.jl_amd/csrc/jg_symbolic.cpp
--- a/juliagrid.jl_amd/csrc/jg_symbolic.cpp
+++ b/juliagrid.jl_amd/csrc/jg_symbolic.cpp
@@ -18,7 +18,7 @@
 
 int knob(const char* name, int unset) {
     static const char* const known[] = {"TRACE", "PLAN_CACHE", "POLL", "PLAN_THREADS", "PLAN_TIMING", "HOST_TIMING",
-                                        "TOP_PW", "TOP_FUSE", "TOP_SYM", "JORDAN", "CHAIN_SMALL", "NO_PREFACTOR", "LANES_INPLACE", "TOP_LEVEL", "ROW_TASKS", "ORDER_CHECK", "TOP_PROFILE", "SINGLE", "SWEEP_ONLY"};
+                                        "TOP_PW", "TOP_FUSE", "TOP_SYM", "JORDAN", "CHAIN_SMALL", "NO_PREFACTOR", "LANES_INPLACE", "TOP_LEVEL", "ROW_TASKS", "ORDER_CHECK", "TOP_PROFILE", "SINGLE", "SWEEP_ONLY", "SWEEP_DEAD"};
     bool ok = false;
     for (const char* k : known) ok = ok || std::strcmp(k, name) == 0;
     if (!ok) return unset;
@@ -1082,6 +1082,13 @@
             }
         }, NoExtra(), 0, 8);
     }
+    out.dead.assign((size_t)n, 1);
+    for (const Rec& r : out.bwd_rec) {
+        if (r.w[0] < 0) continue;
+        for (int t = 0; t < r.w[3] && t < COMP_T; ++t) out.dead[r.w[5 + 2 * t]] = 0;
+    }
+    out.n_dead = out.n_dead_top = 0;
+    for (int r = 0; r < n; ++r) if (out.dead[r]) { out.n_dead++; if (tpos[r] >= 0) out.n_dead_top++; }
 }
 
 void build_single_tables(const BlockSymbolic& S, SingleTables& T) {
@@ -1408,6 +1415,7 @@
     if (S.n_entries + S.n_jordan >= (1 << 24)) S.fact_tasks = 0;
     build_tables(S);
     mark_sweep_dead(S);
+    mark_bwd_dead(S);
     lap("replay tables");
     return 0;
 }
@@ -1485,4 +1493,33 @@
     S.top_dead_blocks *= 2;
 }
 
+void mark_bwd_dead(BlockSymbolic& S) {
+    S.bwd_dead.assign((size_t)S.n, 0);
+    S.bwd_dead_ok = 0; S.bwd_dead_rows = 0;
+    if (!S.jordan || S.symmetric || S.top_task.empty()) return;
+    std::vector<char> named((size_t)S.n, 0);
+    for (const Segment& sg : S.bwdj_seg) {
+        if (sg.wpi <= 0) {
+            for (int x = 0; x < sg.nchunks; ++x) {
+                const Rec& r = S.bwdj_rec[(size_t)sg.rec_base + x];
+                const int nb = r.w[0], nE = r.w[1];
+                const int* d = S.bwd_chain.data() + r.w[2];
+                for (int q = 0; q < nE; ++q) named[d[3 * nb + q]] = 1;
+                const int* uin = d + 3 * nb + nE + nb * nE;
+                for (int p = 0; p < nb; ++p)
+                    for (int c = 0; c < nb; ++c) if (uin[p * nb + c] >= 0) named[d[3 * c]] = 1;
+            }
+            continue;
+        }
+        const size_t nrec = (size_t)sg.nchunks * 16 * sg.rpw;
+        for (size_t x = 0; x < nrec; ++x) {
+            const Rec& r = S.bwdj_rec[(size_t)sg.rec_base + x];
+            if (r.w[0] < 0) continue;
+            for (int t = 0; t < r.w[3] && t < BWD_T; ++t) named[r.w[5 + 2 * t]] = 1;
+        }
+    }
+    S.bwd_dead_ok = 1;
+    for (int k = 0; k < S.n; ++k) if (!named[k]) { S.bwd_dead[k] = 1; S.bwd_dead_rows++; }
 }
+
+}
diff --git a/juliagrid.jl_amd/csrc/jg_symbolic.hpp b/juliagrid.jl_amd/csrc/jg_symbolic.hpp
--- a/juliagrid.jl_amd/csrc/jg_symbolic.hpp
+++ b/juliagrid.jl_amd/csrc/jg_symbolic.hpp
@@ -89,7 +89,12 @@
     int top_dead_ok = 0;
     long long top_dead_blocks = 0;
     long long top_store_blocks = 0;
+    std::vector<char> bwd_dead;
+    int bwd_dead_ok = 0;
+    int bwd_dead_rows = 0;
 };
+constexpr int BWD_DEAD_BIT = 30;
+constexpr int BWD_ENTRY_MASK = 0x3fffffff;
 
 constexpr int COMP_T = 6;
 struct CompTables {
@@ -99,6 +104,8 @@
     std::vector<Segment> fwd_seg, bwd_seg;
     std::vector<Rec> fwd_rec, bwd_rec;
     int n_fwd_levels = 0, n_bwd_levels = 0;
+    std::vector<char> dead;
+    int n_dead = 0, n_dead_top = 0;
 };
 void build_comp_tables(const BlockSymbolic& S, int top_cap, CompTables& out);
 
@@ -121,6 +128,7 @@
 
 int analyze(int n, const int* rowptr, const int* col, long long policy, BlockSymbolic& out);
 void build_selected_inverse(BlockSymbolic& S);
+void mark_bwd_dead(BlockSymbolic& S);
 void mark_sweep_dead(BlockSymbolic& S);
 int entry_of(const BlockSymbolic& S, int r, int c);
 
```

Measured after the change: 413,000, median of 6. 1.03x the previous value.
